# LabJunBMI/E3-invaraint-diffusion-model

Hardware: NVIDIA B200
Metric: denoiser graph-steps/s (forward + reverse-diffusion step per pocket graph; cfg2: 64 pockets x 500 steps, L=128) (higher is better)
Workload: dtype bf16

## Files before the change

e3-invaraint-diffusion-model_b200/csrc/kernels.h:

```cpp
#pragma once
#include "common.cuh"
#include "philox.cuh"

namespace seqdiff {

struct LnResid {
  const float2* stats;
  const float* g;
  const float* b;
};
struct LnOut {
  const float* g;
  const float* b;
  float eps;
  void* h;
  float2* stats;
};
int gemm_16(int M, int N, int K, const void* A, int a_fmt, const void* W, int w_fmt, const float* bias, const float* resid, int epi,
            void* C, int out_kind, cudaStream_t s, int force_bn = 0, const LnResid* ln_resid = nullptr, const LnOut* ln_out = nullptr,
            int split_k = 1);
int gemm_16_tn(int M, int N, int K, const void* At, const void* Bt, int fmt, const float* bias, float* C, cudaStream_t s, int split_k = 1);
int gemm_f32(int M, int N, int K, const float* A, const float* W, const float* bias, const float* resid, int epi, float* C,
             cudaStream_t s);

int make_tmap(const void* ptr, int fmt, int rows, int cols, int box_rows, CUtensorMap* out);
int make_tmap_3d(const void* ptr, int fmt, int batch, int rows, int cols, int box_rows, CUtensorMap* out);

int timestep_embed(const float* timestep, const int* step_ptr, const float* W, int B, int H, float* out, void* out16, int fmt16,
                   cudaStream_t s);
struct EmbedJob {
  const float* x;
  const float* Wt;
  const float* b;
  const float* lnw;
  const float* lnb;
  const float* te;
  float* out32;
  void* outT;
  int M, fin, L;
  const int* src_rows;
  const int* row_graph;
  int cta_begin, cta_count;
};
struct EmbedJobs {
  EmbedJob j[4];
  int n;
  int max_fin;
  float* cat_dst;
  const float* cat_a;
  const float* cat_b;
  int cat_na, cat_nb;
};
template <typename T> int embed_ln_multi(EmbedJobs jobs, float eps, int H, cudaStream_t s);
template <typename T>
int layernorm(const float* in, int M, int H, const float* w, const float* b, float eps, float* out32, T* outT, float2* stats, cudaStream_t s);
template <typename T>
int ln_modulate(const float* in, int M, int H, bool affine_first, const float* lnw, const float* lnb, float eps1, const float* x,
                const T* mod, int mod_div, int chunk0, float* out32, T* outT, cudaStream_t s, const int* row_graph = nullptr);
template <typename T>
int predictor_tail(const T* y, int M, int H, const float* lnw, const float* lnb, float eps, const float* W2, const float* b2,
                   int F, float* logits, cudaStream_t s, const int* dst_rows = nullptr);
template <typename T> int f32_to_16(const float* in, size_t n, T* out, cudaStream_t s);
int transpose_f32(const float* in, int rows, int cols, float* out, cudaStream_t s);
int step_advance(int* step_ptr, cudaStream_t s);

struct AttnPack {
  const int* q_off;
  const int* k_off;
  const int* q_len;
  int q_rows, k_rows;
  int Lk_mask;
};
template <typename T>
int attention(int B, int heads, int Lq, int Lk, const T* q, int ldq, const T* k, int ldk, const T* v, int ldv, const T* dist_emb,
              int P, const float* key_mask, T* out, cudaStream_t s, const AttnPack* pack = nullptr);

int collate(int G, const int* offsets, const uint8_t* lig_mask, const uint8_t* poc_mask, const float* ang, const float* aa, int ext, int L,
            float* lig_ang, float* lig_seq, float* lig_attn, float* rec_ang, float* rec_seq, float* rec_attn, int* lengths, cudaStream_t s);

template <typename T>
int attention_tc(int B, int heads, int Lq, int Lk, const T* q, int ldq, const T* k, int ldk, const T* v, int ldv, const T* dist_emb,
                 int P, const float* key_mask, T* out, cudaStream_t s);
extern unsigned long long* g_attn_trace;
template <typename T>
int attention_pipe(int B, int heads, int Lq, int Lk, const T* q, int ldq, const T* k, int ldk, const T* v, int ldv, const T* dist_emb,
                   int P, const float* key_mask, T* out, cudaStream_t s, const AttnPack* pack = nullptr);
bool attention_bwd_pipe_usable(int Lq, int Lk, const void* dist_emb, float p_drop);
template <typename T>
int attention_bwd_pipe(int B, int heads, int Lq, int Lk, const T* q, int ldq, const T* k, int ldk, const T* v, int ldv, const T* dist_emb, int P,
                       const float* key_mask, DropSpec dr, const T* dout, T* dq, int lddq, T* dk, int lddk, T* dv, int lddv, float* dE, cudaStream_t s,
                       const uint32_t* keep_in = nullptr);
template <typename T>
int attention_pipe_dropout(int B, int heads, int Lq, int Lk, const T* q, int ldq, const T* k, int ldk, const T* v, int ldv, const T* dist_emb,
                           int P, const float* key_mask, DropSpec dr, T* out, cudaStream_t s, uint32_t* keep_out = nullptr);


int reverse_step(const float* q_tables, int n_tab, int B, int L, const float* x_t, const float* logits, int diverse,
                 const float* noise_E, uint64_t seed, uint64_t graph_id0, uint32_t step, const int* step_ptr, float* x_s,
                 uint8_t* idx_out, cudaStream_t s, int* advance = nullptr, const uint64_t* rng = nullptr);
int apply_aa_noise(const float* qtb, int B, int L, const float* x0, const float* noise_E, uint64_t seed, uint64_t graph_id0,
                   uint32_t step, float* x_t, uint8_t* idx_out, cudaStream_t s);
int philox_u32(uint64_t seed, uint64_t graph_id0, uint32_t step, int B, int L, uint32_t* out, cudaStream_t s);

int decode_sequences(int B, int L, const float* final_seq, const float* true_seq, const float* mask, uint8_t* pred_idx, uint8_t* true_idx,
                     int* counts, cudaStream_t s);
int loss_terms(int N, const float* logits, const float* x0, const float* x_t, const float* mask, double* terms, cudaStream_t s,
               double* scratch = nullptr);
size_t loss_terms_scratch_bytes();

int gauss_step(const float* coef, int T, int B, int per_graph, const float* x_t, const float* model_out, const float* noise, uint64_t seed,
               uint64_t graph_id0, int step, const int* step_ptr, float* x_out, float* steps_out, cudaStream_t s, int* advance = nullptr, bool wrap = true,
               const uint64_t* rng = nullptr);

template <typename T> int colsum_add(const T* in, int rows, int cols, float* colsum, cudaStream_t s);
template <typename T> int transpose_colsum(const T* in, int rows, int cols, T* out, float* colsum, cudaStream_t s, int pitch = 0);
template <typename T> int transpose_cast(const float* in, int rows, int cols, T* out, cudaStream_t s);
template <typename T> int act_fwd(const T* z, size_t n, int kind, DropSpec dr, T* a, cudaStream_t s);
template <typename T, typename TG> int act_bwd(const TG* da, const T* z, size_t n, int kind, DropSpec dr, T* dz, cudaStream_t s);
int dropout_add(float* d, const float* resid, size_t n, DropSpec dr, cudaStream_t s);
template <typename T> int grad_cast(const float* g, size_t n, DropSpec dr, T* out, cudaStream_t s);
template <typename T>
int dropout_add_layernorm(float* d, const float* resid, DropSpec dr, int M, int H, const float* w, const float* b, float eps, float* out32, T* outT,
                          uint8_t* keep_bits, cudaStream_t s);
int layernorm_bwd(const float* dh, const float* o, int M, int H, const float* gamma, float eps, float* d_o, float* dgamma, float* dbeta,
                  cudaStream_t s);
template <typename T>
int layernorm_bwd_cast(const float* dh, const float* o, int M, int H, const float* gamma, float eps, float* d_o, float* dgamma, float* dbeta,
                       DropSpec dr, const uint8_t* keep_bits, T* gT, float* dbias, cudaStream_t s);
template <typename T>
int ln_modulate_bwd(const float* dout, const float* in, int M, int H, bool affine_first, const float* lnw, const float* lnb, float eps1,
                    const T* mod, int mod_div, int chunk0, float* din, float* sum_out, T* dmodT, float* dmod32, float* dgamma, float* dbeta,
                    cudaStream_t s);
int embed_bwd(const float* dout, const float* x, int M, int fin, int H, const float* Wt, const float* b, const float* gamma, float eps, DropSpec dr,
              float* dW, float* db, float* dgamma, float* dbeta, cudaStream_t s);
template <typename T>
int predictor_tail_bwd(const float* dlogits, const T* y, int M, int H, const float* gamma, const float* beta, float eps, const float* W2, int F,
                       float* dy, float* dW2, float* db2, float* dgamma, float* dbeta, cudaStream_t s);
int loss_bwd(int N, const float* logits, const float* x0, const float* x_t, const double* terms, float* dlogits, cudaStream_t s);
int adamw_step(float* const* d_w, const int64_t* d_off, int n_slots, size_t total, const float* g, float* m, float* v, float grad_scale,
               float max_norm, float lr, float beta1, float beta2, float eps, float wd, int step, double* d_scratch, float* norm_out, cudaStream_t s);
template <typename T>
int attention_train_fwd(int B, int heads, int Lq, int Lk, const T* q, int ldq, const T* k, int ldk, const T* v, int ldv, const T* dist_emb, int P,
                        const float* key_mask, DropSpec dr, T* out, cudaStream_t s);
template <typename T>
int attention_bwd(int B, int heads, int Lq, int Lk, const T* q, int ldq, const T* k, int ldk, const T* v, int ldv, const T* dist_emb, int P,
                  const float* key_mask, DropSpec dr, const T* dout, T* dq, int lddq, T* dk, int lddk, T* dv, int lddv, float* dE, cudaStream_t s);

template <typename T>
int attention_train_fwd_tc(int B, int heads, int Lq, int Lk, const T* q, int ldq, const T* k, int ldk, const T* v, int ldv, const T* dist_emb, int P,
                           const float* key_mask, DropSpec dr, T* out, cudaStream_t s);
template <typename T>
int attention_bwd_tc(int B, int heads, int Lq, int Lk, const T* q, int ldq, const T* k, int ldk, const T* v, int ldv, const T* dist_emb, int P,
                     const float* key_mask, DropSpec dr, const T* dout, T* dq, int lddq, T* dk, int lddk, T* dv, int lddv, float* dE, cudaStream_t s);

}
```

e3-invaraint-diffusion-model_b200/csrc/model.cu:

```cuda
#include "model.cuh"

#include <mutex>
#include <vector>

#include <cstdio>
#include <cstdlib>
#include <cstring>
#include <type_traits>

namespace seqdiff {

static thread_local std::string g_err;
void set_error(const std::string& msg) { g_err = msg; }
const char* last_error() { return g_err.c_str(); }
std::atomic<uint64_t> g_launches{0};

bool g_profiling = false;
struct ProfMark { const char* tag; cudaEvent_t ev; cudaStream_t s; };
static std::vector<ProfMark> g_marks;
void profile_mark(const char* tag, cudaStream_t s) {
  cudaStreamCaptureStatus st = cudaStreamCaptureStatusNone;
  if (cudaStreamIsCapturing(s, &st) != cudaSuccess || st != cudaStreamCaptureStatusNone) return;
  cudaEvent_t ev;
  if (cudaEventCreate(&ev) != cudaSuccess) return;
  cudaEventRecord(ev, s);
  g_marks.push_back({tag, ev, s});
}
int profile_begin(cudaStream_t s) {
  for (auto& m : g_marks) cudaEventDestroy(m.ev);
  g_marks.clear();
  g_profiling = true;
  profile_mark("__begin__", s);
  return SEQDIFF_OK;
}
int profile_end(char* tags, int tag_stride, float* ms, int* counts, int cap) {
  g_profiling = false;
  if (cudaDeviceSynchronize() != cudaSuccess) return -1;
  std::map<std::string, std::pair<double, int>> agg;
  std::map<cudaStream_t, cudaEvent_t> prev;
  for (auto& m : g_marks) {
    auto it = prev.find(m.s);
    if (it != prev.end() && std::string(m.tag) != "__begin__") {
      float t = 0.f;
      if (cudaEventElapsedTime(&t, it->second, m.ev) == cudaSuccess) {
        auto& a = agg[m.tag];
        a.first += t;
        a.second += 1;
      }
    }
    prev[m.s] = m.ev;
  }
  int n = 0;
  for (auto& kv : agg) {
    if (n >= cap) break;
    std::snprintf(tags + static_cast<size_t>(n) * tag_stride, tag_stride, "%s", kv.first.c_str());
    ms[n] = static_cast<float>(kv.second.first);
    counts[n] = kv.second.second;
    ++n;
  }
  for (auto& m : g_marks) cudaEventDestroy(m.ev);
  g_marks.clear();
  return n;
}

static thread_local int g_pdl_scope = 0;
struct PdlScope {
  const int prev;
  explicit PdlScope(int mode = 1) : prev(g_pdl_scope) { if (mode) g_pdl_scope = mode; }
  ~PdlScope() { g_pdl_scope = prev; }
};
int pdl_scope_exchange(int mode) {
  const int prev = g_pdl_scope;
  g_pdl_scope = mode;
  return prev;
}
static int pdl_auto_mode(long long rows) { return rows <= 2048 ? 1 : (rows <= 32768 ? 3 : 0); }
int pdl_mode() {
  static const int env = [] { const char* e = getenv("SEQDIFF_PDL"); return e ? (e[0] >= '0' && e[0] <= '3' ? e[0] - '0' : 0) : -1; }();
  return env >= 0 ? env : g_pdl_scope;
}
bool pdl_enabled() { return pdl_mode() == 1; }

#ifdef SEQDIFF_DEBUG_BOUNDS
namespace {
struct GuardRec { const void* owner; void* p; };
std::vector<GuardRec> g_guards;
std::mutex g_guard_mu;
constexpr uint32_t kGuardWord = 0xA5C3F00Du;
__global__ void guard_fill_kernel(uint32_t* p) { p[threadIdx.x] = kGuardWord; }
__global__ void guard_check_kernel(uint32_t* const* bands, int n, int* broken) {
  const int i = blockIdx.x;
  if (i < n && bands[i][threadIdx.x] != kGuardWord) atomicAdd(broken, 1);
}
}
int debug_guard_begin(const void* owner) {
  std::lock_guard<std::mutex> g(g_guard_mu);
  size_t w = 0;
  for (size_t i = 0; i < g_guards.size(); ++i)
    if (g_guards[i].owner != owner) g_guards[w++] = g_guards[i];
  g_guards.resize(w);
  return SEQDIFF_OK;
}
int debug_guard_add(const void* owner, void* p, cudaStream_t s) {
  {
    std::lock_guard<std::mutex> g(g_guard_mu);
    g_guards.push_back({owner, p});
  }
  guard_fill_kernel<<<1, 64, 0, s>>>(static_cast<uint32_t*>(p));
  SD_CUDA(cudaGetLastError());
  return SEQDIFF_OK;
}
int debug_guard_check(cudaStream_t s, int* n_bands, int* n_broken) {
  std::vector<uint32_t*> h;
  {
    std::lock_guard<std::mutex> g(g_guard_mu);
    for (auto& r : g_guards) h.push_back(static_cast<uint32_t*>(r.p));
  }
  *n_bands = static_cast<int>(h.size());
  *n_broken = 0;
  if (h.empty()) return SEQDIFF_OK;
  SD_CUDA(cudaDeviceSynchronize());
  if (const char* e = getenv("SEQDIFF_DEBUG_BREAK_GUARD"); e && e[0] == '1') SD_CUDA(cudaMemset(h[h.size() / 2], 0, 4));
  uint32_t** d = nullptr;
  int* cnt = nullptr;
  SD_CUDA(cudaMalloc(reinterpret_cast<void**>(&d), h.size() * sizeof(uint32_t*)));
  SD_CUDA(cudaMalloc(reinterpret_cast<void**>(&cnt), sizeof(int)));
  SD_CUDA(cudaMemcpy(d, h.data(), h.size() * sizeof(uint32_t*), cudaMemcpyHostToDevice));
  SD_CUDA(cudaMemset(cnt, 0, sizeof(int)));
  guard_check_kernel<<<static_cast<unsigned>(h.size()), 64, 0, s>>>(d, static_cast<int>(h.size()), cnt);
  SD_CUDA(cudaGetLastError());
  SD_CUDA(cudaStreamSynchronize(s));
  SD_CUDA(cudaMemcpy(n_broken, cnt, sizeof(int), cudaMemcpyDeviceToHost));
  cudaFree(d);
  cudaFree(cnt);
  return SEQDIFF_OK;
}
#else
int debug_guard_begin(const void*) { return SEQDIFF_OK; }
int debug_guard_add(const void*, void*, cudaStream_t) { return SEQDIFF_OK; }
int debug_guard_check(cudaStream_t, int* n_bands, int* n_broken) { *n_bands = 0; *n_broken = 0; return SEQDIFF_OK; }
#endif

int num_sms() {
  static int n = 0;
  if (n == 0) {
    int dev = 0;
    if (cudaGetDevice(&dev) != cudaSuccess || cudaDeviceGetAttribute(&n, cudaDevAttrMultiProcessorCount, dev) != cudaSuccess || n <= 0)
      n = 148;
  }
  return n;
}

template <typename T> struct Fmt;
template <> struct Fmt<f16> { static constexpr int v = 0; };
template <> struct Fmt<bf16> { static constexpr int v = 1; };
template <> struct Fmt<float> { static constexpr int v = -1; };

template <typename T> static const T* pick(const Wt& w);
template <> const float* pick<float>(const Wt& w) { return w.f; }
template <> const bf16* pick<bf16>(const Wt& w) { return w.h; }
template <> const f16* pick<f16>(const Wt& w) { return w.g; }

static int gemm_T(int, int M, int N, int K, const float* A, const Wt& W, const float* bias, int epi, float* C, cudaStream_t s) {
  return gemm_f32(M, N, K, A, W.f, bias, nullptr, epi, C, s);
}
template <typename T>
static int gemm_T(int wfmt, int M, int N, int K, const T* A, const Wt& W, const float* bias, int epi, T* C, cudaStream_t s) {
  const void* w = wfmt == 1 ? static_cast<const void*>(W.h) : static_cast<const void*>(W.g);
  return gemm_16(M, N, K, A, Fmt<T>::v, w, wfmt, bias, nullptr, epi, C, Fmt<T>::v, s);
}
static int gemm_S(int, int M, int N, int K, const float* A, const Wt& W, const float* bias, const float* resid, float* C, cudaStream_t s) {
  return gemm_f32(M, N, K, A, W.f, bias, resid, 0, C, s);
}
template <typename T>
static int gemm_S(int wfmt, int M, int N, int K, const T* A, const Wt& W, const float* bias, const float* resid, float* C, cudaStream_t s,
                  const LnResid* ln = nullptr, const LnOut* lo = nullptr) {
  const void* w = wfmt == 1 ? static_cast<const void*>(W.h) : static_cast<const void*>(W.g);
  return gemm_16(M, N, K, A, Fmt<T>::v, w, wfmt, bias, resid, 0, C, 2, s, 0, ln, lo);
}
static bool ln_fuse_enabled(int H) {
  static const bool on = [] { const char* e = getenv("SEQDIFF_LN_FUSE"); return e && e[0] == '1'; }();
  return on && (H == 512 || H == 768 || H == 1024);
}
template <typename T>
static int gemm_ln(int wfmt, int M, int H, int K, const T* A, const Wt& W, const float* bias, const float* resid, float* o, const LnResid* lr,
                   const float* ln_w, const float* ln_b, float eps, T* h, float2* stats, cudaStream_t s) {
  if (ln_fuse_enabled(H)) {
    const LnOut lo{ln_w, ln_b, eps, h, stats};
    return gemm_S(wfmt, M, H, K, A, W, bias, resid, o, s, lr, &lo);
  }
  SD_TRY(gemm_S(wfmt, M, H, K, A, W, bias, resid, o, s, lr));
  return layernorm<T>(o, M, H, ln_w, ln_b, eps, nullptr, h, stats, s);
}

__global__ void set_int_kernel(int* p, int v) {
  pdl_trigger();
  pdl_wait();
  *p = v;
}
__global__ void arm_loop_kernel(int* step, int v, uint64_t* rng, uint64_t seed, uint64_t gid0) {
  pdl_trigger();
  pdl_wait();
  step[0] = v;
  step[1] = 0;
  rng[0] = seed;
  rng[1] = gid0;
}

Model::~Model() {
  if (graph_exec) cudaGraphExecDestroy(graph_exec);
  if (loop_stream) cudaStreamDestroy(loop_stream);
  if (ev_in) cudaEventDestroy(ev_in);
  if (ev_out) cudaEventDestroy(ev_out);
  for (void* p : allocs) cudaFree(p);
  for (void* p : packed_allocs) cudaFree(p);
  if (ws) { debug_guard_begin(ws); cudaFree(ws); }
  if (samp_in) { debug_guard_begin(samp_in); cudaFree(samp_in); }
  if (d_tables) cudaFree(d_tables);
  if (d_pack) cudaFree(d_pack);
  if (tws) { debug_guard_begin(tws); cudaFree(tws); }
  if (d_rp_tables) cudaFree(d_rp_tables);
}

void* Model::dalloc(size_t bytes) {
  if (packing && repack_reuse) {
    if (packed_cursor < packed_allocs.size()) return packed_allocs[packed_cursor++];
    return nullptr;
  }
  void* p = nullptr;
  if (cudaMalloc(&p, bytes < 256 ? 256 : bytes) != cudaSuccess) return nullptr;
  (packing ? packed_allocs : allocs).push_back(p);
  return p;
}

static void add_schema(std::map<std::string, RawTensor>& raw, const std::string& name, int64_t numel) {
  RawTensor t;
  t.numel = numel;
  raw[name] = t;
}

int Model::init(const seqdiff_config_t& c, int dev, int arch_) {
  cfg = c;
  device = dev;
  arch = arch_;
  SD_CHECK(c.hidden_size % 256 == 0 && c.hidden_size >= 256 && c.hidden_size <= 1024, "hidden_size must be 256/512/768/1024");
  SD_CHECK(c.num_attention_heads * 64 == c.hidden_size, "head_dim must be 64");
  SD_CHECK(c.intermediate_size % 128 == 0, "intermediate_size must be a multiple of 128");
  SD_CHECK(c.num_hidden_layers >= 1 && c.max_position_embeddings >= 1, "bad layer count / max positions");
  SD_CHECK(c.feature_size >= 1 && c.feature_size <= 32, "feature_size must be in [1,32]");
  SD_CUDA(cudaSetDevice(dev));
  const int64_t H = c.hidden_size, I = c.intermediate_size, P = c.max_position_embeddings;
  add_schema(raw, "timestep_projector.W", H / 2);
  auto emb_schema = [&](const std::string& p, int fin) {
    add_schema(raw, p + ".linear.weight", H * fin);
    add_schema(raw, p + ".linear.bias", H);
    add_schema(raw, p + ".LayerNorm.weight", H);
    add_schema(raw, p + ".LayerNorm.bias", H);
  };
  if (arch == kArchSequence)
    for (const char* side : {"ligand", "receptor"})
      for (auto kv : {std::pair<const char*, int>{"seq", 20}, std::pair<const char*, int>{"angle", 8}})
        emb_schema(std::string(side) + "_" + kv.first + "_embedding", kv.second);
  auto attn = [&](const std::string& p, bool rel) {
    for (const char* n : {"query", "key", "value"}) {
      add_schema(raw, p + ".self." + n + ".weight", H * H);
      add_schema(raw, p + ".self." + n + ".bias", H);
    }
    if (rel && c.relative_key) add_schema(raw, p + ".self.distance_embedding.weight", (2 * P - 1) * 64);
    add_schema(raw, p + ".output.dense.weight", H * H);
    add_schema(raw, p + ".output.dense.bias", H);
    add_schema(raw, p + ".output.LayerNorm.weight", H);
    add_schema(raw, p + ".output.LayerNorm.bias", H);
  };
  auto ffn_schema = [&](const std::string& p) {
    add_schema(raw, p + ".intermediate.dense.weight", I * H);
    add_schema(raw, p + ".intermediate.dense.bias", I);
    add_schema(raw, p + ".output.dense.weight", H * I);
    add_schema(raw, p + ".output.dense.bias", H);
    add_schema(raw, p + ".output.LayerNorm.weight", H);
    add_schema(raw, p + ".output.LayerNorm.bias", H);
  };
  const std::vector<const char*> se_blocks = arch == kArchSequence
                                                 ? std::vector<const char*>{"ligand_feature_emb", "receptor_feature_emb", "decoder_normalize"}
                                                 : std::vector<const char*>{"receptor_emb", "timestep_emb"};
  for (const char* blk : se_blocks) {
    const std::string p = blk;
    add_schema(raw, p + ".adaLN_modulation.0.weight", H * H);
    add_schema(raw, p + ".adaLN_modulation.0.bias", H);
    add_schema(raw, p + ".adaLN_modulation.2.weight", 6 * H * H);
    add_schema(raw, p + ".adaLN_modulation.2.bias", 6 * H);
    attn(p + ".attn", true);
    add_schema(raw, p + ".mlp.0.weight", 4 * H * H);
    add_schema(raw, p + ".mlp.0.bias", 4 * H);
    add_schema(raw, p + ".mlp.3.weight", 4 * H * H);
    add_schema(raw, p + ".mlp.3.bias", H);
  }
  for (int i = 0; i < c.num_hidden_layers; ++i) {
    const std::string p = "decoder.layer." + std::to_string(i);
    attn(p + ".attention", true);
    attn(p + ".crossattention", false);
    ffn_schema(p);
  }
  if (arch == kArchStructure) {
    emb_schema("receptor_seq_emb", 20);
    emb_schema("receptor_angle_emb", c.feature_size);
    emb_schema("ligand_angle_emb", c.feature_size);
    for (int i = 0; i < c.num_hidden_layers; ++i) {
      const std::string p = "encoder.layer." + std::to_string(i);
      attn(p + ".attention", true);
      ffn_schema(p);
    }
  }
  const std::string head = arch == kArchSequence ? "amino_acid_predictor" : "angles_predictor";
  add_schema(raw, head + ".dense1.weight", H * H);
  add_schema(raw, head + ".dense1.bias", H);
  add_schema(raw, head + ".layer_norm.weight", H);
  add_schema(raw, head + ".layer_norm.bias", H);
  add_schema(raw, head + ".dense2.weight", static_cast<int64_t>(c.feature_size) * H);
  add_schema(raw, head + ".dense2.bias", c.feature_size);
  d_step = static_cast<int*>(dalloc(256));
  SD_CHECK(d_step != nullptr, "cudaMalloc failed");
  SD_CUDA(cudaMemset(d_step, 0, 256));
  return SEQDIFF_OK;
}

int Model::set_tensor(const char* name, const float* data, int64_t numel, cudaStream_t s) {
  auto it = raw.find(name);
  if (it == raw.end()) {
    set_error(std::string("unknown tensor name: ") + name);
    return SEQDIFF_ERR_STATE;
  }
  RawTensor& t = it->second;
  if (t.numel != numel) {
    set_error(std::string("size mismatch for ") + name + ": expected " + std::to_string(t.numel) + ", got " + std::to_string(numel));
    return SEQDIFF_ERR_INVALID;
  }
  if (arch == kArchSequence && std::strncmp(name, "receptor_feature_emb.", 21) == 0) {
    t.set = true;
    return SEQDIFF_OK;
  }
  if (!t.ptr) {
    t.ptr = static_cast<float*>(dalloc(static_cast<size_t>(numel) * sizeof(float)));
    SD_CHECK(t.ptr != nullptr, "cudaMalloc failed");
  }
  SD_CUDA(cudaMemcpyAsync(t.ptr, data, static_cast<size_t>(numel) * sizeof(float), cudaMemcpyDefault, s));
  t.set = true;
  finalized = false;
  return SEQDIFF_OK;
}

namespace {
struct RpChunk { const float* src; void* a; void* b; int n, rows, cols, r0; };
__global__ void __launch_bounds__(256) rp_copy_kernel(const RpChunk* __restrict__ tab) {
  const RpChunk c = tab[blockIdx.x];
  float* dst = static_cast<float*>(c.a);
  for (int i = threadIdx.x * 4; i < c.n; i += 1024) {
    if (i + 3 < c.n) *reinterpret_cast<float4*>(dst + i) = *reinterpret_cast<const float4*>(c.src + i);
    else for (int j = i; j < c.n; ++j) dst[j] = c.src[j];
  }
}
__global__ void __launch_bounds__(256) rp_conv_kernel(const RpChunk* __restrict__ tab) {
  const RpChunk c = tab[blockIdx.x];
  bf16* h = static_cast<bf16*>(c.a);
  f16* g = static_cast<f16*>(c.b);
  for (int i = threadIdx.x * 4; i < c.n; i += 1024) {
    if (i + 3 < c.n) {
      const float4 v = *reinterpret_cast<const float4*>(c.src + i);
      *reinterpret_cast<uint2*>(h + i) = make_uint2(pack_bf16x2(v.x, v.y), pack_bf16x2(v.z, v.w));
      *reinterpret_cast<uint2*>(g + i) = make_uint2(pack_f16x2(v.x, v.y), pack_f16x2(v.z, v.w));
    } else {
      for (int j = i; j < c.n; ++j) { h[j] = from_f32<bf16>(c.src[j]); g[j] = from_f32<f16>(c.src[j]); }
    }
  }
}
template <typename T>
__global__ void __launch_bounds__(256) rp_trans_kernel(const RpChunk* __restrict__ tab) {
  __shared__ float tile[64][65];
  const RpChunk c = tab[blockIdx.x];
  T* out = static_cast<T*>(c.a);
  const int r0 = c.r0, c0 = c.n;
  const int tx = threadIdx.x & 63, ty = threadIdx.x >> 6;
#pragma unroll 4
  for (int i = ty; i < 64; i += 4) {
    const int r = r0 + i, cc = c0 + tx;
    tile[i][tx] = (r < c.rows && cc < c.cols) ? c.src[static_cast<size_t>(r) * c.cols + cc] : 0.f;
  }
  __syncthreads();
#pragma unroll 4
  for (int i = ty; i < 64; i += 4) {
    const int cc = c0 + i, r = r0 + tx;
    if (cc < c.cols && r < c.rows) out[static_cast<size_t>(cc) * c.rows + r] = from_f32<T>(tile[tx][i]);
  }
}
}

int Model::repack_fast(cudaStream_t s) {
  constexpr int kChunk = 8192;
  if (!d_rp_tables || rp_table_prec != train_prec) {
    std::vector<RpChunk> tab;
    for (const RpCopy& o : rp_copy)
      for (int64_t off = 0; off < o.n; off += kChunk)
        tab.push_back({o.src + off, o.dst + off, nullptr, static_cast<int>(o.n - off < kChunk ? o.n - off : kChunk), 0, 0, 0});
    rp_n_copy = static_cast<int>(tab.size());
    for (const RpConv& o : rp_conv)
      for (int64_t off = 0; off < o.n; off += kChunk)
        tab.push_back({o.src + off, static_cast<bf16*>(o.h) + off, static_cast<f16*>(o.g) + off, static_cast<int>(o.n - off < kChunk ? o.n - off : kChunk), 0, 0, 0});
    rp_n_conv = static_cast<int>(tab.size()) - rp_n_copy;
    auto tiles = [&](const std::vector<RpTrans>& ops) {
      for (const RpTrans& o : ops)
        for (int r0 = 0; r0 < o.rows; r0 += 64)
          for (int c0 = 0; c0 < o.cols; c0 += 64) tab.push_back({o.src, o.dst, nullptr, c0, o.rows, o.cols, r0});
    };
    const size_t before = tab.size();
    tiles(rp_trans);
    rp_n_trans = static_cast<int>(tab.size() - before);
    tiles(rp_trans_f32);
    rp_n_trans_f32 = static_cast<int>(tab.size() - before) - rp_n_trans;
    if (d_rp_tables) { SD_CUDA(cudaDeviceSynchronize()); SD_CUDA(cudaFree(d_rp_tables)); d_rp_tables = nullptr; }
    SD_CUDA(cudaMalloc(&d_rp_tables, tab.size() * sizeof(RpChunk)));
    SD_CUDA(cudaMemcpyAsync(d_rp_tables, tab.data(), tab.size() * sizeof(RpChunk), cudaMemcpyHostToDevice, s));
    SD_CUDA(cudaStreamSynchronize(s));
    rp_table_prec = train_prec;
  }
  const RpChunk* t = static_cast<const RpChunk*>(d_rp_tables);
  if (rp_n_copy) { SD_CUDA(launch_k(rp_copy_kernel, dim3(rp_n_copy), dim3(256), 0, s, t)); SD_LAUNCHED("repack_copy", s); }
  t += rp_n_copy;
  if (rp_n_conv) { SD_CUDA(launch_k(rp_conv_kernel, dim3(rp_n_conv), dim3(256), 0, s, t)); SD_LAUNCHED("repack_convert", s); }
  t += rp_n_conv;
  if (rp_n_trans) {
    if (train_prec == SEQDIFF_FP32) SD_CUDA(launch_k(rp_trans_kernel<float>, dim3(rp_n_trans), dim3(256), 0, s, t));
    else if (train_prec == SEQDIFF_BF16) SD_CUDA(launch_k(rp_trans_kernel<bf16>, dim3(rp_n_trans), dim3(256), 0, s, t));
    else SD_CUDA(launch_k(rp_trans_kernel<f16>, dim3(rp_n_trans), dim3(256), 0, s, t));
    SD_LAUNCHED("repack_transpose", s);
  }
  t += rp_n_trans;
  if (rp_n_trans_f32) { SD_CUDA(launch_k(rp_trans_kernel<float>, dim3(rp_n_trans_f32), dim3(256), 0, s, t)); SD_LAUNCHED("repack_transpose", s); }
  return SEQDIFF_OK;
}

int Model::finalize(cudaStream_t s) {
  for (auto& kv : raw)
    if (!kv.second.set) {
      set_error("tensor never set: " + kv.first);
      return SEQDIFF_ERR_STATE;
    }
  if (!repack_reuse) {
    if (graph_exec) {
      cudaGraphExecDestroy(graph_exec);
      graph_exec = nullptr;
      graph_key = GraphKey();
    }
    if (!packed_allocs.empty()) {
      SD_CUDA(cudaDeviceSynchronize());
      for (void* p : packed_allocs) cudaFree(p);
      packed_allocs.clear();
    }
  }
  if (repack_reuse && !rp_conv.empty()) return repack_fast(s);
  packed_cursor = 0;
  packing = true;
  rp_copy.clear(); rp_conv.clear(); rp_trans.clear(); rp_trans_f32.clear();
  rp_table_prec = -2;
  const int64_t H = cfg.hidden_size, I = cfg.intermediate_size, P = cfg.max_position_embeddings;
  int rc = SEQDIFF_OK;
  auto R = [&](const std::string& n) -> const float* { return raw.at(n).ptr; };
  auto transposed = [&](Wt& w, int64_t rows, int64_t cols) {
    w.rows = rows;
    w.cols = cols;
    if (train_prec < 0) return;
    const size_t n = static_cast<size_t>(rows) * cols;
    void* t = dalloc(n * (train_prec == SEQDIFF_FP32 ? 4 : 2));
    int r = SEQDIFF_ERR_CUDA;
    if (t) {
      if (train_prec == SEQDIFF_FP32) r = transpose_cast<float>(w.f, static_cast<int>(rows), static_cast<int>(cols), static_cast<float*>(t), s);
      else if (train_prec == SEQDIFF_BF16) r = transpose_cast<bf16>(w.f, static_cast<int>(rows), static_cast<int>(cols), static_cast<bf16*>(t), s);
      else r = transpose_cast<f16>(w.f, static_cast<int>(rows), static_cast<int>(cols), static_cast<f16*>(t), s);
    }
    if (r != SEQDIFF_OK) rc = SEQDIFF_ERR_CUDA;
    w.t = t;
    rp_trans.push_back({w.f, t, static_cast<int>(rows), static_cast<int>(cols)});
  };
  auto both = [&](const float* f, int64_t n) -> Wt {
    Wt w;
    w.f = f;
    bf16* h = static_cast<bf16*>(dalloc(static_cast<size_t>(n) * sizeof(bf16)));
    f16* g = static_cast<f16*>(dalloc(static_cast<size_t>(n) * sizeof(f16)));
    if (!h || !g || f32_to_16<bf16>(f, static_cast<size_t>(n), h, s) != SEQDIFF_OK ||
        f32_to_16<f16>(f, static_cast<size_t>(n), g, s) != SEQDIFF_OK)
      rc = SEQDIFF_ERR_CUDA;
    w.h = h;
    w.g = g;
    rp_conv.push_back({f, h, g, n});
    return w;
  };
  auto stack = [&](const std::vector<const float*>& parts, int64_t each) -> float* {
    float* dst = static_cast<float*>(dalloc(parts.size() * static_cast<size_t>(each) * sizeof(float)));
    if (!dst) { rc = SEQDIFF_ERR_CUDA; return nullptr; }
    for (size_t i = 0; i < parts.size(); ++i) {
      if (cudaMemcpyAsync(dst + i * each, parts[i], static_cast<size_t>(each) * sizeof(float), cudaMemcpyDeviceToDevice, s) != cudaSuccess)
        rc = SEQDIFF_ERR_CUDA;
      rp_copy.push_back({dst + i * each, parts[i], each});
    }
    return dst;
  };
  auto emb = [&](const std::string& p, int fin) -> EmbW {
    EmbW e;
    e.fin = fin;
    float* wt = static_cast<float*>(dalloc(static_cast<size_t>(H) * fin * sizeof(float)));
    if (!wt || transpose_f32(R(p + ".linear.weight"), static_cast<int>(H), fin, wt, s) != SEQDIFF_OK) rc = SEQDIFF_ERR_CUDA;
    e.Wt_ = wt;
    rp_trans_f32.push_back({R(p + ".linear.weight"), wt, static_cast<int>(H), fin});
    e.b = R(p + ".linear.bias");
    e.ln_w = R(p + ".LayerNorm.weight");
    e.ln_b = R(p + ".LayerNorm.bias");
    return e;
  };
  auto attn = [&](const std::string& p, bool self_rel) -> AttnW {
    AttnW a;
    const float* w = stack({R(p + ".self.query.weight"), R(p + ".self.key.weight"), R(p + ".self.value.weight")}, H * H);
    a.qkv = both(w, 3 * H * H);
    transposed(a.qkv, 3 * H, H);
    a.qkv_b = stack({R(p + ".self.query.bias"), R(p + ".self.key.bias"), R(p + ".self.value.bias")}, H);
    if (self_rel && cfg.relative_key) a.E = both(R(p + ".self.distance_embedding.weight"), (2 * P - 1) * 64);
    a.out = both(R(p + ".output.dense.weight"), H * H);
    transposed(a.out, H, H);
    a.out_b = R(p + ".output.dense.bias");
    a.ln_w = R(p + ".output.LayerNorm.weight");
    a.ln_b = R(p + ".output.LayerNorm.bias");
    return a;
  };
  auto se = [&](const std::string& p) -> SEW {
    SEW w;
    w.ada0 = both(R(p + ".adaLN_modulation.0.weight"), H * H);
    transposed(w.ada0, H, H);
    w.ada0_b = R(p + ".adaLN_modulation.0.bias");
    w.ada2 = both(R(p + ".adaLN_modulation.2.weight"), 6 * H * H);
    transposed(w.ada2, 6 * H, H);
    w.ada2_b = R(p + ".adaLN_modulation.2.bias");
    w.attn = attn(p + ".attn", true);
    w.m0 = both(R(p + ".mlp.0.weight"), 4 * H * H);
    transposed(w.m0, 4 * H, H);
    w.m0_b = R(p + ".mlp.0.bias");
    w.m3 = both(R(p + ".mlp.3.weight"), 4 * H * H);
    transposed(w.m3, H, 4 * H);
    w.m3_b = R(p + ".mlp.3.bias");
    return w;
  };
  ts_W = R("timestep_projector.W");
  auto ffn = [&](const std::string& p, LayerW& l) {
    l.inter = both(R(p + ".intermediate.dense.weight"), I * H);
    transposed(l.inter, I, H);
    l.inter_b = R(p + ".intermediate.dense.bias");
    l.outd = both(R(p + ".output.dense.weight"), H * I);
    transposed(l.outd, H, I);
    l.outd_b = R(p + ".output.dense.bias");
    l.oln_w = R(p + ".output.LayerNorm.weight");
    l.oln_b = R(p + ".output.LayerNorm.bias");
  };
  enc_layers.clear();
  if (arch == kArchSequence) {
    lig_seq = emb("ligand_seq_embedding", 20);
    lig_ang = emb("ligand_angle_embedding", 8);
    rec_seq = emb("receptor_seq_embedding", 20);
    rec_ang = emb("receptor_angle_embedding", 8);
    se_lig = se("ligand_feature_emb");
    se_dec = se("decoder_normalize");
  } else {
    rec_seq = emb("receptor_seq_emb", 20);
    rec_ang = emb("receptor_angle_emb", cfg.feature_size);
    lig_ang = emb("ligand_angle_emb", cfg.feature_size);
    se_lig = se("receptor_emb");
    se_dec = se("timestep_emb");
    for (int i = 0; i < cfg.num_hidden_layers; ++i) {
      const std::string p = "encoder.layer." + std::to_string(i);
      LayerW l;
      l.self = attn(p + ".attention", true);
      ffn(p, l);
      enc_layers.push_back(l);
    }
  }
  layers.clear();
  std::vector<const float*> ckv_w, ckv_b;
  for (int i = 0; i < cfg.num_hidden_layers; ++i) {
    const std::string p = "decoder.layer." + std::to_string(i);
    LayerW l;
    l.self = attn(p + ".attention", true);
    l.cq = both(R(p + ".crossattention.self.query.weight"), H * H);
    transposed(l.cq, H, H);
    l.cq_b = R(p + ".crossattention.self.query.bias");
    ckv_w.push_back(R(p + ".crossattention.self.key.weight"));
    ckv_w.push_back(R(p + ".crossattention.self.value.weight"));
    ckv_b.push_back(R(p + ".crossattention.self.key.bias"));
    ckv_b.push_back(R(p + ".crossattention.self.value.bias"));
    l.cout = both(R(p + ".crossattention.output.dense.weight"), H * H);
    transposed(l.cout, H, H);
    l.cout_b = R(p + ".crossattention.output.dense.bias");
    l.cln_w = R(p + ".crossattention.output.LayerNorm.weight");
    l.cln_b = R(p + ".crossattention.output.LayerNorm.bias");
    ffn(p, l);
    layers.push_back(l);
  }
  ckv_all = both(stack(ckv_w, H * H), static_cast<int64_t>(ckv_w.size()) * H * H);
  transposed(ckv_all, static_cast<int64_t>(ckv_w.size()) * H, H);
  ckv_all_b = stack(ckv_b, H);
  const std::string head = arch == kArchSequence ? "amino_acid_predictor" : "angles_predictor";
  p1 = both(R(head + ".dense1.weight"), H * H);
  transposed(p1, H, H);
  p1_b = R(head + ".dense1.bias");
  p_ln_w = R(head + ".layer_norm.weight");
  p_ln_b = R(head + ".layer_norm.bias");
  p2_w = R(head + ".dense2.weight");
  p2_b = R(head + ".dense2.bias");
  packing = false;
  if (rc != SEQDIFF_OK) {
    set_error("finalize: allocation or packing kernel failed");
    return rc;
  }
  finalized = true;
  return SEQDIFF_OK;
}

static size_t align256(size_t b) { return (b + 255) & ~static_cast<size_t>(255); }

size_t Model::workspace_need(int precision, int B, int Ll, int Lr) const {
  const size_t es = precision == SEQDIFF_FP32 ? 4 : 2;
  const size_t dual = precision == SEQDIFF_FP32 ? 4 : 4 + 2;
  const size_t H = cfg.hidden_size, I = cfg.intermediate_size, NL = cfg.num_hidden_layers;
  const size_t Ml = static_cast<size_t>(B) * Ll, Mr = static_cast<size_t>(B) * Lr, Mt = Ml + Mr;
  size_t n = 0;
  n += 2 * align256(static_cast<size_t>(B) * H * 4);
  n += align256((Ml + Mr) * 4);
  n += 3 * (align256(Mt * H * 4) + align256(Mt * H * 2));
  n += 2 * align256(Mt * H * 4);
  n += 3 * align256(Mt * H * es);
  n += align256(Mt * 6 * H * es);
  n += align256(Mt * 3 * H * es);
  n += align256(Mt * 4 * H * es);
  n += align256(Mr * NL * 2 * H * es);
  n += 2 * (align256(Ml * H * 4) + align256(Ml * H * 2));
  n += 2 * align256(Ml * H * es);
  n += align256(Ml * H * 4) + align256(Ml * 3 * 8);
  n += align256(Ml * I * es);
  (void)dual;
  return n + 8192 + 64 * kGuardBytes;
}

int Model::ensure_workspace(size_t bytes) {
  if (bytes <= ws_bytes) return SEQDIFF_OK;
  if (ws) {
    SD_CUDA(cudaDeviceSynchronize());
    debug_guard_begin(ws);
    SD_CUDA(cudaFree(ws));
    ws = nullptr;
    ws_bytes = 0;
  }
  SD_CUDA(cudaMalloc(reinterpret_cast<void**>(&ws), bytes));
  ws_bytes = bytes;
  return SEQDIFF_OK;
}

struct Bump {
  uint8_t* p;
  cudaStream_t gs;
  const void* owner;
  explicit Bump(uint8_t* base, cudaStream_t s = nullptr) : p(base), gs(s), owner(base) { debug_guard_begin(owner); }
  template <typename T> T* take(size_t n) {
    T* r = reinterpret_cast<T*>(p);
    p += align256(n * sizeof(T));
    if (kGuardBytes) {
      debug_guard_add(owner, p, gs);
      p += kGuardBytes;
    }
    return r;
  }
};

template <typename T> struct Act {
  float* s = nullptr;
  T* t = nullptr;
  T* t_out() const { return t; }
};
template <> struct Act<float> {
  float* s = nullptr;
  float* t = nullptr;
  float* t_out() const { return nullptr; }
};
template <typename T> static Act<T> take_act(Bump& bp, size_t n) {
  Act<T> a;
  a.s = bp.take<float>(n);
  a.t = bp.take<T>(n);
  return a;
}
template <> Act<float> take_act<float>(Bump& bp, size_t n) {
  Act<float> a;
  a.s = bp.take<float>(n);
  a.t = a.s;
  return a;
}
template <typename T> static Act<T> offset(const Act<T>& a, size_t n) {
  Act<T> r;
  r.s = a.s + n;
  r.t = a.t + n;
  return r;
}

template <typename T> struct SEBufs {
  T *u, *mod, *qkv, *ctx, *m1;
  float *o, *m2;
  Act<T> x1;
};

template <typename T>
static int se_layer(const Model& m, int wfmt, const SEW& w, const Act<T>& x, const T* c, int Mc, int mod_div, int M,
                    const std::vector<Segment>& segs, const SEBufs<T>& b, const Act<T>& out, cudaStream_t s,
                    const std::vector<AttnPack>* packs = nullptr, const int* row_graph = nullptr) {
  const int H = m.cfg.hidden_size, P = m.cfg.max_position_embeddings, heads = m.cfg.num_attention_heads;
  SD_TRY(gemm_T(wfmt, Mc, H, H, c, w.ada0, w.ada0_b, 2, b.u, s));
  SD_TRY(gemm_T(wfmt, Mc, 6 * H, H, b.u, w.ada2, w.ada2_b, 0, b.mod, s));
  SD_TRY(gemm_T(wfmt, M, 3 * H, H, x.t, w.attn.qkv, w.attn.qkv_b, 0, b.qkv, s));
  for (size_t gi = 0; gi < segs.size(); ++gi) {
    const Segment& g = segs[gi];
    const T* base = b.qkv + static_cast<size_t>(g.row0) * 3 * H;
    SD_TRY(attention<T>(g.B, heads, g.L, g.L, base, 3 * H, base + H, 3 * H, base + 2 * H, 3 * H, pick<T>(w.attn.E), P, g.mask,
                        b.ctx + static_cast<size_t>(g.row0) * H, s, packs ? &(*packs)[gi] : nullptr));
  }
  SD_TRY(gemm_S(wfmt, M, H, H, b.ctx, w.attn.out, w.attn.out_b, x.s, b.o, s));
  SD_TRY(ln_modulate<T>(b.o, M, H, true, w.attn.ln_w, w.attn.ln_b, m.cfg.layer_norm_eps, x.s, b.mod, mod_div, 0, b.x1.s, b.x1.t_out(), s, row_graph));
  SD_TRY(gemm_T(wfmt, M, 4 * H, H, b.x1.t, w.m0, w.m0_b, 1, b.m1, s));
  SD_TRY(gemm_S(wfmt, M, H, 4 * H, b.m1, w.m3, w.m3_b, nullptr, b.m2, s));
  SD_TRY(ln_modulate<T>(b.m2, M, H, false, nullptr, nullptr, 0.f, b.x1.s, b.mod, mod_div, 3, out.s, out.t_out(), s, row_graph));
  return SEQDIFF_OK;
}


template <typename T>
int Model::forward_t(int wfmt, int B, int Ll, int Lr, const float* timestep, const int* step_ptr, const float* x_t,
                     const float* lig_angle, const float* lig_mask, const float* rec_seq_in, const float* rec_angle,
                     const float* rec_mask, float* logits, cudaStream_t s, const PackInfo* pk) {
  constexpr bool k16 = !std::is_same<T, float>::value;
  const int H = cfg.hidden_size, I = cfg.intermediate_size, NL = cfg.num_hidden_layers, heads = cfg.num_attention_heads;
  const int P = cfg.max_position_embeddings;
  const float eps = cfg.layer_norm_eps;
  const int Ml = pk ? pk->Ml : B * Ll, Mr = pk ? pk->Mr : B * Lr, Mt = Ml + Mr;
  const int Mlp = B * Ll, Mrp = B * Lr;
  const size_t MtH = static_cast<size_t>(Mt) * H, MlH = static_cast<size_t>(Ml) * H;
  Bump bp(ws, s);
  float* te = bp.take<float>(static_cast<size_t>(B) * H);
  T* teT = k16 ? bp.take<T>(static_cast<size_t>(B) * H) : reinterpret_cast<T*>(te);
  float* maskcat = bp.take<float>(static_cast<size_t>(Mlp) + Mrp);
  Act<T> x = take_act<T>(bp, MtH);
  Act<T> x2 = take_act<T>(bp, MtH);
  SEBufs<T> sb;
  sb.x1 = take_act<T>(bp, MtH);
  sb.o = bp.take<float>(MtH);
  sb.m2 = bp.take<float>(MtH);
  T* ccat = bp.take<T>(MtH);
  sb.u = bp.take<T>(MtH);
  sb.ctx = bp.take<T>(MtH);
  sb.mod = bp.take<T>(MtH * 6);
  sb.qkv = bp.take<T>(MtH * 3);
  sb.m1 = bp.take<T>(MtH * 4);
  T* kv_all = bp.take<T>(static_cast<size_t>(Mr) * NL * 2 * H);
  Act<T> hbuf[2] = {take_act<T>(bp, MlH), take_act<T>(bp, MlH)};
  float* obuf3 = bp.take<float>(MlH);
  float2* lnstats = bp.take<float2>(3 * static_cast<size_t>(Ml));
  T* cq = bp.take<T>(MlH);
  T* y = bp.take<T>(MlH);
  T* ffn = bp.take<T>(static_cast<size_t>(Ml) * I);

  SD_TRY(timestep_embed(timestep, step_ptr, ts_W, B, H, te, k16 ? static_cast<void*>(teT) : nullptr, Fmt<T>::v, s));
  const Act<T> xr = offset(x, MlH);
  {
    auto job = [&](const float* in, int M, const EmbW& e, const float* te_, int L, float* o32, T* oT, bool lig) {
      EmbedJob jb{};
      jb.x = in; jb.Wt = e.Wt_; jb.b = e.b; jb.lnw = e.ln_w; jb.lnb = e.ln_b; jb.te = te_;
      jb.out32 = o32; jb.outT = oT; jb.M = M; jb.fin = e.fin; jb.L = L;
      if (pk) {
        jb.src_rows = lig ? pk->src_l : pk->src_r;
        jb.row_graph = lig ? pk->graph : pk->graph + pk->Ml;
      }
      return jb;
    };
    EmbedJobs jobs{};
    jobs.n = 4;
    jobs.j[0] = job(x_t, Ml, lig_seq, nullptr, Ll, x.s, x.t_out(), true);
    jobs.j[1] = job(rec_seq_in, Mr, rec_seq, nullptr, Lr, xr.s, xr.t_out(), false);
    jobs.j[2] = job(lig_angle, Ml, lig_ang, te, Ll, k16 ? nullptr : reinterpret_cast<float*>(ccat), k16 ? ccat : nullptr, true);
    jobs.j[3] = job(rec_angle, Mr, rec_ang, te, Lr, k16 ? nullptr : reinterpret_cast<float*>(ccat + MlH), k16 ? ccat + MlH : nullptr, false);
    if (Ll == Lr) {
      jobs.cat_dst = maskcat; jobs.cat_a = lig_mask; jobs.cat_b = rec_mask; jobs.cat_na = Mlp; jobs.cat_nb = Mrp;
    }
    SD_TRY(embed_ln_multi<T>(jobs, eps, H, s));
  }

  std::vector<Segment> segs;
  std::vector<AttnPack> packs;
  AttnPack pk_self{}, pk_cross{};
  if (pk) {
    if (Ll == Lr) {
      segs.push_back({0, 2 * B, pk->max_l > pk->max_r ? pk->max_l : pk->max_r, maskcat});
      packs.push_back(AttnPack{pk->off_cat, pk->off_cat, pk->len_cat, Mt, Mt, Ll});
    } else {
      segs.push_back({0, B, pk->max_l, lig_mask});
      packs.push_back(AttnPack{pk->off_cat, pk->off_cat, pk->len_cat, Mt, Mt, Ll});
      segs.push_back({0, B, pk->max_r, rec_mask});
      packs.push_back(AttnPack{pk->off_cat + B, pk->off_cat + B, pk->len_cat + B, Mt, Mt, Lr});
    }
    pk_self = AttnPack{pk->off_l, pk->off_l, pk->len_l, Ml, Ml, Ll};
    pk_cross = AttnPack{pk->off_l, pk->off_r, pk->len_l, Ml, Mr, Lr};
  } else if (Ll == Lr) {
    segs.push_back({0, 2 * B, Ll, maskcat});
  } else {
    segs.push_back({0, B, Ll, lig_mask});
    segs.push_back({Ml, B, Lr, rec_mask});
  }
  const int Lq_self = pk ? pk->max_l : Ll, Lk_cross = pk ? pk->max_r : Lr;
  const AttnPack* aps = pk ? &pk_self : nullptr;
  const AttnPack* apc = pk ? &pk_cross : nullptr;
  SD_TRY(se_layer<T>(*this, wfmt, se_lig, x, ccat, Mt, 1, Mt, segs, sb, x2, s, pk ? &packs : nullptr, nullptr));
  const T* rec = x2.t + MlH;

  SD_TRY(gemm_T(wfmt, Mr, NL * 2 * H, H, rec, ckv_all, ckv_all_b, 0, kv_all, s));
  Act<T> h = x2;
  if constexpr (k16) {
    float* obuf[3] = {sb.o, sb.m2, obuf3};
    LnResid prev{};
    const float* o_prev = nullptr;
    for (int i = 0; i < NL; ++i) {
      const LayerW& w = layers[i];
      const bool last = i + 1 == NL;
      const Act<T> h1 = hbuf[0], h2 = hbuf[1], h3 = hbuf[0];
      float* oA = obuf[0];
      float* oB = obuf[1];
      float* oC = obuf[2];
      SD_TRY(gemm_T(wfmt, Ml, 3 * H, H, h.t, w.self.qkv, w.self.qkv_b, 0, sb.qkv, s));
      SD_TRY(attention<T>(B, heads, Lq_self, Lq_self, sb.qkv, 3 * H, sb.qkv + H, 3 * H, sb.qkv + 2 * H, 3 * H, pick<T>(w.self.E), P, lig_mask, sb.ctx, s, aps));
      SD_TRY(gemm_ln<T>(wfmt, Ml, H, H, sb.ctx, w.self.out, w.self.out_b, i == 0 ? h.s : o_prev, oA, i == 0 ? nullptr : &prev, w.self.ln_w,
                        w.self.ln_b, eps, h1.t, lnstats, s));
      SD_TRY(gemm_T(wfmt, Ml, H, H, h1.t, w.cq, w.cq_b, 0, cq, s));
      const T* kbase = kv_all + static_cast<size_t>(i) * 2 * H;
      SD_TRY(attention<T>(B, heads, Lq_self, Lk_cross, cq, H, kbase, NL * 2 * H, kbase + H, NL * 2 * H, static_cast<const T*>(nullptr), P, rec_mask, sb.ctx, s, apc));
      const LnResid r1{lnstats, w.self.ln_w, w.self.ln_b};
      SD_TRY(gemm_ln<T>(wfmt, Ml, H, H, sb.ctx, w.cout, w.cout_b, oA, oB, &r1, w.cln_w, w.cln_b, eps, h2.t, lnstats + Ml, s));
      SD_TRY(gemm_T(wfmt, Ml, I, H, h2.t, w.inter, w.inter_b, 1, ffn, s));
      const LnResid r2{lnstats + Ml, w.cln_w, w.cln_b};
      if (last) {
        SD_TRY(gemm_S(wfmt, Ml, H, I, ffn, w.outd, w.outd_b, oB, oC, s, &r2));
        SD_TRY(layernorm<T>(oC, Ml, H, w.oln_w, w.oln_b, eps, h3.s, h3.t, lnstats + 2 * static_cast<size_t>(Ml), s));
      } else {
        SD_TRY(gemm_ln<T>(wfmt, Ml, H, I, ffn, w.outd, w.outd_b, oB, oC, &r2, w.oln_w, w.oln_b, eps, h3.t, lnstats + 2 * static_cast<size_t>(Ml), s));
      }
      prev = LnResid{lnstats + 2 * static_cast<size_t>(Ml), w.oln_w, w.oln_b};
      o_prev = oC;
      h = h3;
    }
  } else {
    for (int i = 0; i < NL; ++i) {
      const LayerW& w = layers[i];
      const Act<T> h1 = hbuf[0], h2 = hbuf[1], h3 = hbuf[0];
      SD_TRY(gemm_T(wfmt, Ml, 3 * H, H, h.t, w.self.qkv, w.self.qkv_b, 0, sb.qkv, s));
      SD_TRY(attention<T>(B, heads, Lq_self, Lq_self, sb.qkv, 3 * H, sb.qkv + H, 3 * H, sb.qkv + 2 * H, 3 * H, pick<T>(w.self.E), P, lig_mask, sb.ctx, s, aps));
      SD_TRY(gemm_S(wfmt, Ml, H, H, sb.ctx, w.self.out, w.self.out_b, h.s, sb.o, s));
      SD_TRY(layernorm<T>(sb.o, Ml, H, w.self.ln_w, w.self.ln_b, eps, h1.s, h1.t_out(), nullptr, s));
      SD_TRY(gemm_T(wfmt, Ml, H, H, h1.t, w.cq, w.cq_b, 0, cq, s));
      const T* kbase = kv_all + static_cast<size_t>(i) * 2 * H;
      SD_TRY(attention<T>(B, heads, Lq_self, Lk_cross, cq, H, kbase, NL * 2 * H, kbase + H, NL * 2 * H, static_cast<const T*>(nullptr), P, rec_mask, sb.ctx, s, apc));
      SD_TRY(gemm_S(wfmt, Ml, H, H, sb.ctx, w.cout, w.cout_b, h1.s, sb.o, s));
      SD_TRY(layernorm<T>(sb.o, Ml, H, w.cln_w, w.cln_b, eps, h2.s, h2.t_out(), nullptr, s));
      SD_TRY(gemm_T(wfmt, Ml, I, H, h2.t, w.inter, w.inter_b, 1, ffn, s));
      SD_TRY(gemm_S(wfmt, Ml, H, I, ffn, w.outd, w.outd_b, h2.s, sb.o, s));
      SD_TRY(layernorm<T>(sb.o, Ml, H, w.oln_w, w.oln_b, eps, h3.s, h3.t_out(), nullptr, s));
      h = h3;
    }
  }

  std::vector<Segment> lseg{{0, B, Lq_self, lig_mask}};
  std::vector<AttnPack> lpack;
  if (pk) lpack.push_back(pk_self);
  SD_TRY(se_layer<T>(*this, wfmt, se_dec, h, teT, B, Ll, Ml, lseg, sb, x, s, pk ? &lpack : nullptr, pk ? pk->graph : nullptr));

  if constexpr (std::is_same<T, bf16>::value) {
    f16* xh = reinterpret_cast<f16*>(sb.ctx);
    f16* yh = reinterpret_cast<f16*>(y);
    SD_TRY(f32_to_16<f16>(x.s, static_cast<size_t>(Ml) * H, xh, s));
    SD_TRY(gemm_16(Ml, H, H, xh, 0, p1.g, 0, p1_b, nullptr, 1, yh, 0, s));
    SD_TRY(predictor_tail<f16>(yh, Ml, H, p_ln_w, p_ln_b, 1e-12f, p2_w, p2_b, cfg.feature_size, logits, s, pk ? pk->src_l : nullptr));
    return SEQDIFF_OK;
  }
  SD_TRY(gemm_T(wfmt, Ml, H, H, x.t, p1, p1_b, 1, y, s));
  SD_TRY(predictor_tail<T>(y, Ml, H, p_ln_w, p_ln_b, 1e-12f, p2_w, p2_b, cfg.feature_size, logits, s, pk ? pk->src_l : nullptr));
  return SEQDIFF_OK;
}

int Model::forward(int precision, int B, int Ll, int Lr, const float* timestep, const int* step_ptr, const float* x_t,
                   const float* lig_angle, const float* lig_mask, const float* rec_seq_in, const float* rec_angle,
                   const float* rec_mask, float* logits, cudaStream_t s, const PackInfo* pk) {
  SD_CHECK(finalized, "model not finalised (seqdiff_model_finalize)");
  SD_CHECK(arch == kArchSequence, "handle holds a structure model: use seqdiff_struct_forward");
  SD_CHECK(!pk || precision != SEQDIFF_FP32, "ragged packing runs in the 16-bit modes");
  SD_CHECK(precision >= SEQDIFF_FP32 && precision <= SEQDIFF_FP16, "unknown precision mode");
  SD_CHECK(B > 0 && Ll > 0 && Lr > 0, "empty batch");
  if (cfg.relative_key) SD_CHECK(Ll <= cfg.max_position_embeddings && Lr <= cfg.max_position_embeddings, "Length exceed");
  SD_CUDA(cudaSetDevice(device));
  SD_TRY(ensure_workspace(workspace_need(precision, B, Ll, Lr)));
  if (g_profiling) profile_mark("__begin__", s);
  const PdlScope pdl_scope(pdl_auto_mode(pk ? static_cast<long long>(pk->Ml) + pk->Mr : static_cast<long long>(B) * (Ll + Lr)));
  switch (precision) {
    case SEQDIFF_FP32:
      return forward_t<float>(1, B, Ll, Lr, timestep, step_ptr, x_t, lig_angle, lig_mask, rec_seq_in, rec_angle, rec_mask, logits, s, nullptr);
    case SEQDIFF_BF16:
      return forward_t<bf16>(1, B, Ll, Lr, timestep, step_ptr, x_t, lig_angle, lig_mask, rec_seq_in, rec_angle, rec_mask, logits, s, pk);
    default:
      return forward_t<f16>(0, B, Ll, Lr, timestep, step_ptr, x_t, lig_angle, lig_mask, rec_seq_in, rec_angle, rec_mask, logits, s, pk);
  }
}

int Model::build_pack(int B, int Ll, int Lr, const float* lig_mask, const float* rec_mask, cudaStream_t s, bool* usable) {
  *usable = false;
  std::vector<float> hl(static_cast<size_t>(B) * Ll), hr(static_cast<size_t>(B) * Lr);
  SD_CUDA(cudaMemcpyAsync(hl.data(), lig_mask, hl.size() * 4, cudaMemcpyDefault, s));
  SD_CUDA(cudaMemcpyAsync(hr.data(), rec_mask, hr.size() * 4, cudaMemcpyDefault, s));
  SD_CUDA(cudaStreamSynchronize(s));
  std::vector<int> len_l(B), len_r(B);
  auto lengths = [&](const std::vector<float>& m, int L, std::vector<int>& len) -> bool {
    for (int b = 0; b < B; ++b) {
      int n = 0;
      while (n < L && m[static_cast<size_t>(b) * L + n] == 1.0f) ++n;
      for (int i = n; i < L; ++i)
        if (m[static_cast<size_t>(b) * L + i] != 0.0f) return false;
      if (n == 0) return false;
      len[b] = n;
    }
    return true;
  };
  if (!lengths(hl, Ll, len_l) || !lengths(hr, Lr, len_r)) return SEQDIFF_OK;
  int Ml = 0, Mr = 0, max_l = 0, max_r = 0;
  std::vector<int> off_l(B), off_r(B);
  for (int b = 0; b < B; ++b) {
    off_l[b] = Ml; Ml += len_l[b];
    off_r[b] = Mr; Mr += len_r[b];
    max_l = len_l[b] > max_l ? len_l[b] : max_l;
    max_r = len_r[b] > max_r ? len_r[b] : max_r;
  }
  std::vector<int> blk;
  blk.reserve(2 * (static_cast<size_t>(Ml) + Mr) + 8 * B);
  for (int b = 0; b < B; ++b) for (int l = 0; l < len_l[b]; ++l) blk.push_back(b * Ll + l);
  for (int b = 0; b < B; ++b) for (int l = 0; l < len_r[b]; ++l) blk.push_back(b * Lr + l);
  for (int b = 0; b < B; ++b) for (int l = 0; l < len_l[b]; ++l) blk.push_back(b);
  for (int b = 0; b < B; ++b) for (int l = 0; l < len_r[b]; ++l) blk.push_back(b);
  for (int b = 0; b < B; ++b) blk.push_back(off_l[b]);
  for (int b = 0; b < B; ++b) blk.push_back(off_r[b]);
  for (int b = 0; b < B; ++b) blk.push_back(len_l[b]);
  for (int b = 0; b < B; ++b) blk.push_back(len_r[b]);
  for (int b = 0; b < B; ++b) blk.push_back(off_l[b]);
  for (int b = 0; b < B; ++b) blk.push_back(Ml + off_r[b]);
  for (int b = 0; b < B; ++b) blk.push_back(len_l[b]);
  for (int b = 0; b < B; ++b) blk.push_back(len_r[b]);
  uint64_t hsh = 1469598103934665603ull;
  for (int v : blk) { hsh ^= static_cast<uint32_t>(v); hsh *= 1099511628211ull; }
  bool fresh = false;
  if (blk.size() > pack_cap) {
    if (d_pack) { SD_CUDA(cudaDeviceSynchronize()); SD_CUDA(cudaFree(d_pack)); d_pack = nullptr; pack_cap = 0; }
    SD_CUDA(cudaMalloc(reinterpret_cast<void**>(&d_pack), blk.size() * sizeof(int)));
    pack_cap = blk.size();
    fresh = true;
  }
  if (fresh || hsh != pack.hash || pack.B != B) {
    SD_CUDA(cudaMemcpyAsync(d_pack, blk.data(), blk.size() * sizeof(int), cudaMemcpyHostToDevice, s));
    SD_CUDA(cudaStreamSynchronize(s));
  }
  PackInfo pi;
  pi.B = B; pi.Ml = Ml; pi.Mr = Mr; pi.max_l = max_l; pi.max_r = max_r; pi.hash = hsh;
  const int* p = d_pack;
  pi.src_l = p; p += Ml;
  pi.src_r = p; p += Mr;
  pi.graph = p; p += Ml + Mr;
  pi.off_l = p; p += B;
  pi.off_r = p; p += B;
  pi.len_l = p; p += B;
  pi.len_r = p; p += B;
  pi.off_cat = p; p += 2 * B;
  pi.len_cat = p;
  pack = pi;
  *usable = true;
  return SEQDIFF_OK;
}

int Model::sample(int precision, int B, int Ll, int Lr, int T, const float* q_tables, const float* x_T, const float* lig_angle,
                  const float* lig_mask, const float* rec_seq_in, const float* rec_angle, const float* rec_mask, int diverse,
                  const float* noise_E, uint64_t seed, uint64_t gid0, float* final_out, cudaStream_t caller, int flags) {
  SD_CHECK(finalized, "model not finalised (seqdiff_model_finalize)");
  SD_CHECK(T >= 1 && B > 0 && Ll > 0 && Lr > 0, "bad sampling arguments");
  SD_CHECK(cfg.feature_size == SEQDIFF_NUM_CLASSES, "sampling needs feature_size == 20");
  SD_CUDA(cudaSetDevice(device));
  if (!loop_stream) {
    SD_CUDA(cudaStreamCreateWithFlags(&loop_stream, cudaStreamNonBlocking));
    SD_CUDA(cudaEventCreateWithFlags(&ev_in, cudaEventDisableTiming));
    SD_CUDA(cudaEventCreateWithFlags(&ev_out, cudaEventDisableTiming));
  }
  cudaStream_t s = loop_stream;
  SD_CUDA(cudaEventRecord(ev_in, caller));
  SD_CUDA(cudaStreamWaitEvent(s, ev_in, 0));
  const size_t Nl = static_cast<size_t>(B) * Ll, Nr = static_cast<size_t>(B) * Lr;
  const size_t need_in = align256(Nl * 20 * 4) * 2 + align256(Nl * 8 * 4) + align256(Nl * 4) + align256(Nr * 20 * 4) +
                         align256(Nr * 8 * 4) + align256(Nr * 4);
  if (need_in + 16 * kGuardBytes > samp_in_bytes) {
    if (samp_in) { SD_CUDA(cudaDeviceSynchronize()); debug_guard_begin(samp_in); SD_CUDA(cudaFree(samp_in)); samp_in = nullptr; samp_in_bytes = 0; }
    SD_CUDA(cudaMalloc(reinterpret_cast<void**>(&samp_in), need_in + 16 * kGuardBytes));
    samp_in_bytes = need_in + 16 * kGuardBytes;
  }
  const size_t tab_floats = static_cast<size_t>(T) * 3 * 400;
  if (tab_floats > tables_cap) {
    if (d_tables) { SD_CUDA(cudaDeviceSynchronize()); SD_CUDA(cudaFree(d_tables)); d_tables = nullptr; tables_cap = 0; }
    SD_CUDA(cudaMalloc(reinterpret_cast<void**>(&d_tables), tab_floats * 4));
    tables_cap = tab_floats;
  }
  SD_TRY(ensure_workspace(workspace_need(precision, B, Ll, Lr)));
  Bump bp(samp_in, s);
  float* x_cur = bp.take<float>(Nl * 20);
  float* logits = bp.take<float>(Nl * 20);
  float* c_lang = bp.take<float>(Nl * 8);
  float* c_lmask = bp.take<float>(Nl);
  float* c_rseq = bp.take<float>(Nr * 20);
  float* c_rang = bp.take<float>(Nr * 8);
  float* c_rmask = bp.take<float>(Nr);
  SD_CUDA(cudaMemcpyAsync(d_tables, q_tables, tab_floats * 4, cudaMemcpyDefault, s));
  SD_CUDA(cudaMemcpyAsync(x_cur, x_T, Nl * 20 * 4, cudaMemcpyDefault, s));
  SD_CUDA(cudaMemcpyAsync(c_lang, lig_angle, Nl * 8 * 4, cudaMemcpyDefault, s));
  SD_CUDA(cudaMemcpyAsync(c_lmask, lig_mask, Nl * 4, cudaMemcpyDefault, s));
  SD_CUDA(cudaMemcpyAsync(c_rseq, rec_seq_in, Nr * 20 * 4, cudaMemcpyDefault, s));
  SD_CUDA(cudaMemcpyAsync(c_rang, rec_angle, Nr * 8 * 4, cudaMemcpyDefault, s));
  SD_CUDA(cudaMemcpyAsync(c_rmask, rec_mask, Nr * 4, cudaMemcpyDefault, s));
  const PackInfo* pk = nullptr;
  if ((flags & 1) && precision != SEQDIFF_FP32) {
    bool usable = false;
    SD_TRY(build_pack(B, Ll, Lr, c_lmask, c_rmask, s, &usable));
    if (usable) {
      pk = &pack;
      SD_CUDA(cudaMemsetAsync(logits, 0, Nl * 20 * 4, s));
    }
  }

  GraphKey key;
  key.pack_hash = pk ? pk->hash : 0;
  key.precision = precision; key.B = B; key.Ll = Ll; key.Lr = Lr; key.diverse = diverse; key.noise = noise_E;
  key.ws_ptr = ws; key.in_ptr = samp_in; key.tab_ptr = d_tables;
  uint64_t* d_rng = reinterpret_cast<uint64_t*>(d_step + 16);
  auto one_step = [&](cudaStream_t st) -> int {
    const PdlScope pdl_scope(pdl_auto_mode(pk ? static_cast<long long>(pk->Ml) + pk->Mr : static_cast<long long>(B) * (Ll + Lr)));
    SD_TRY(forward(precision, B, Ll, Lr, nullptr, d_step, x_cur, c_lang, c_lmask, c_rseq, c_rang, c_rmask, logits, st, pk));
    SD_TRY(reverse_step(d_tables, 1, B, Ll, x_cur, logits, diverse, noise_E, 0, 0, 0, d_step, x_cur, nullptr, st, d_step + 1, d_rng));
    return SEQDIFF_OK;
  };
  if (!graph_exec || !(key == graph_key)) {
    if (graph_exec) { cudaGraphExecDestroy(graph_exec); graph_exec = nullptr; }
    SD_CUDA(launch_k(set_int_kernel, dim3(1), dim3(1), 0, s, d_step, T - 1));
    SD_LAUNCHED("set_int", s);
    SD_TRY(forward(precision, B, Ll, Lr, nullptr, d_step, x_cur, c_lang, c_lmask, c_rseq, c_rang, c_rmask, logits, s, pk));
    SD_CUDA(cudaStreamSynchronize(s));
    cudaGraph_t graph = nullptr;
    const uint64_t l0 = g_launches.load();
    SD_CUDA(cudaStreamBeginCapture(s, cudaStreamCaptureModeThreadLocal));
    const int rc = one_step(s);
    graph_kernels = static_cast<int>(g_launches.load() - l0);
    cudaError_t ce = cudaStreamEndCapture(s, &graph);
    if (rc != SEQDIFF_OK) { if (graph) cudaGraphDestroy(graph); return rc; }
    SD_CUDA(ce);
    ce = cudaGraphInstantiate(&graph_exec, graph, 0);
    cudaGraphDestroy(graph);
    SD_CUDA(ce);
    graph_key = key;
  }
  SD_CUDA(launch_k(arm_loop_kernel, dim3(1), dim3(1), 0, s, d_step, T - 1, d_rng, seed, gid0));
  SD_LAUNCHED("arm_loop", s);
  for (int it = 0; it < T; ++it) SD_CUDA(cudaGraphLaunch(graph_exec, s));
  g_launches.fetch_add(static_cast<uint64_t>(T) * graph_kernels, std::memory_order_relaxed);
  SD_CUDA(cudaMemcpyAsync(final_out, logits, Nl * 20 * 4, cudaMemcpyDefault, s));
  SD_CUDA(cudaEventRecord(ev_out, s));
  SD_CUDA(cudaStreamWaitEvent(caller, ev_out, 0));
  return SEQDIFF_OK;
}

template <typename T>
static int bert_layer_plain(const Model& m, int wfmt, const LayerW& w, bool cross, int B, int Lq, int Lk, const Act<T>& h, const float* q_mask,
                            const float* k_mask, const T* kbase, int ldkv, T* qkv, T* ctx, T* cq, T* ffn, float* o, const Act<T>& h1,
                            const Act<T>& h2, Act<T>* out, cudaStream_t s) {
  const int H = m.cfg.hidden_size, I = m.cfg.intermediate_size, heads = m.cfg.num_attention_heads, P = m.cfg.max_position_embeddings;
  const float eps = m.cfg.layer_norm_eps;
  const int M = B * Lq;
  SD_TRY(gemm_T(wfmt, M, 3 * H, H, h.t, w.self.qkv, w.self.qkv_b, 0, qkv, s));
  SD_TRY(attention<T>(B, heads, Lq, Lq, qkv, 3 * H, qkv + H, 3 * H, qkv + 2 * H, 3 * H, pick<T>(w.self.E), P, q_mask, ctx, s));
  SD_TRY(gemm_S(wfmt, M, H, H, ctx, w.self.out, w.self.out_b, h.s, o, s));
  SD_TRY(layernorm<T>(o, M, H, w.self.ln_w, w.self.ln_b, eps, h1.s, h1.t_out(), nullptr, s));
  Act<T> cur = h1, nxt = h2;
  if (cross) {
    SD_TRY(gemm_T(wfmt, M, H, H, h1.t, w.cq, w.cq_b, 0, cq, s));
    SD_TRY(attention<T>(B, heads, Lq, Lk, cq, H, kbase, ldkv, kbase + H, ldkv, static_cast<const T*>(nullptr), P, k_mask, ctx, s));
    SD_TRY(gemm_S(wfmt, M, H, H, ctx, w.cout, w.cout_b, h1.s, o, s));
    SD_TRY(layernorm<T>(o, M, H, w.cln_w, w.cln_b, eps, h2.s, h2.t_out(), nullptr, s));
    cur = h2;
    nxt = h1;
  }
  SD_TRY(gemm_T(wfmt, M, I, H, cur.t, w.inter, w.inter_b, 1, ffn, s));
  SD_TRY(gemm_S(wfmt, M, H, I, ffn, w.outd, w.outd_b, cur.s, o, s));
  SD_TRY(layernorm<T>(o, M, H, w.oln_w, w.oln_b, eps, nxt.s, nxt.t_out(), nullptr, s));
  *out = nxt;
  return SEQDIFF_OK;
}

template <typename T>
static int bert_stack_lnresid(const Model& m, int wfmt, const std::vector<LayerW>& Ls, bool cross, int B, int Lq, int Lk, const Act<T>& h0,
                              const float* q_mask, const float* k_mask, const T* kv_all, int ldkv, T* qkv, T* ctx, T* cq, T* ffn,
                              float* const (&obuf)[3], float2* lnstats, T* hT0, T* hT1, const T** out, cudaStream_t s) {
  const int H = m.cfg.hidden_size, I = m.cfg.intermediate_size, heads = m.cfg.num_attention_heads, P = m.cfg.max_position_embeddings;
  const float eps = m.cfg.layer_norm_eps;
  const int M = B * Lq;
  float2* stA = lnstats;
  float2* stB = lnstats + M;
  float2* stC = lnstats + 2 * static_cast<size_t>(M);
  LnResid prev{};
  const float* o_prev = nullptr;
  const T* h = h0.t;
  for (size_t i = 0; i < Ls.size(); ++i) {
    const LayerW& w = Ls[i];
    SD_TRY(gemm_T(wfmt, M, 3 * H, H, h, w.self.qkv, w.self.qkv_b, 0, qkv, s));
    SD_TRY(attention<T>(B, heads, Lq, Lq, qkv, 3 * H, qkv + H, 3 * H, qkv + 2 * H, 3 * H, pick<T>(w.self.E), P, q_mask, ctx, s));
    SD_TRY(gemm_ln<T>(wfmt, M, H, H, ctx, w.self.out, w.self.out_b, i == 0 ? h0.s : o_prev, obuf[0], i == 0 ? nullptr : &prev, w.self.ln_w,
                      w.self.ln_b, eps, hT0, stA, s));
    const T* cur = hT0;
    const float* o_cur = obuf[0];
    LnResid rc{stA, w.self.ln_w, w.self.ln_b};
    if (cross) {
      SD_TRY(gemm_T(wfmt, M, H, H, hT0, w.cq, w.cq_b, 0, cq, s));
      const T* kbase = kv_all + i * 2 * static_cast<size_t>(H);
      SD_TRY(attention<T>(B, heads, Lq, Lk, cq, H, kbase, ldkv, kbase + H, ldkv, static_cast<const T*>(nullptr), P, k_mask, ctx, s));
      SD_TRY(gemm_ln<T>(wfmt, M, H, H, ctx, w.cout, w.cout_b, obuf[0], obuf[1], &rc, w.cln_w, w.cln_b, eps, hT1, stB, s));
      cur = hT1;
      o_cur = obuf[1];
      rc = LnResid{stB, w.cln_w, w.cln_b};
    }
    SD_TRY(gemm_T(wfmt, M, I, H, cur, w.inter, w.inter_b, 1, ffn, s));
    T* nxt = cross ? hT0 : hT1;
    SD_TRY(gemm_ln<T>(wfmt, M, H, I, ffn, w.outd, w.outd_b, o_cur, obuf[2], &rc, w.oln_w, w.oln_b, eps, nxt, stC, s));
    prev = LnResid{stC, w.oln_w, w.oln_b};
    o_prev = obuf[2];
    h = nxt;
  }
  *out = h;
  return SEQDIFF_OK;
}

size_t Model::struct_workspace_need(int precision, int B, int Ll, int Lr) const {
  const size_t es = precision == SEQDIFF_FP32 ? 4 : 2;
  const size_t H = cfg.hidden_size, I = cfg.intermediate_size, NL = cfg.num_hidden_layers;
  const size_t Mr = static_cast<size_t>(B) * Lr, Mx = static_cast<size_t>(B) * (Ll > Lr ? Ll : Lr);
  size_t n = align256(Mr * NL * 2 * H * es);
  n += 2 * align256(static_cast<size_t>(B) * H * 4);
  n += 5 * (align256(Mx * H * 4) + align256(Mx * H * 2));
  n += 2 * align256(Mx * H * 4);
  n += 5 * align256(Mx * H * es);
  n += align256(Mx * 6 * H * es) + align256(Mx * 3 * H * es) + align256(Mx * 4 * H * es);
  n += align256(Mx * I * es);
  return n + 8192 + 64 * kGuardBytes;
}

template <typename T>
int Model::struct_forward_t(int wfmt, int B, int Ll, int Lr, const float* timestep, const int* step_ptr, const float* noised,
                            const float* lig_mask, const float* rec_seq_in, const float* rec_angle, const float* rec_mask, float* out,
                            int phases, cudaStream_t s) {
  constexpr bool k16 = !std::is_same<T, float>::value;
  const int H = cfg.hidden_size, I = cfg.intermediate_size, NL = cfg.num_hidden_layers;
  const float eps = cfg.layer_norm_eps;
  const int Ml = B * Ll, Mr = B * Lr, Mx = Ml > Mr ? Ml : Mr;
  const size_t MxH = static_cast<size_t>(Mx) * H;
  Bump bp(ws, s);
  T* kv_all = bp.take<T>(static_cast<size_t>(Mr) * NL * 2 * H);
  float* te = bp.take<float>(static_cast<size_t>(B) * H);
  T* teT = k16 ? bp.take<T>(static_cast<size_t>(B) * H) : reinterpret_cast<T*>(te);
  Act<T> x = take_act<T>(bp, MxH);
  Act<T> x2 = take_act<T>(bp, MxH);
  SEBufs<T> sb;
  sb.x1 = take_act<T>(bp, MxH);
  Act<T> hb[2] = {take_act<T>(bp, MxH), take_act<T>(bp, MxH)};
  sb.o = bp.take<float>(MxH);
  sb.m2 = bp.take<float>(MxH);
  T* cT = bp.take<T>(MxH);
  sb.u = bp.take<T>(MxH);
  sb.ctx = bp.take<T>(MxH);
  T* cq = bp.take<T>(MxH);
  T* y = bp.take<T>(MxH);
  sb.mod = bp.take<T>(MxH * 6);
  sb.qkv = bp.take<T>(MxH * 3);
  sb.m1 = bp.take<T>(MxH * 4);
  T* ffn = bp.take<T>(static_cast<size_t>(Mx) * I);
  auto job = [&](const float* in, int M, const EmbW& e, int L, float* o32, T* oT) {
    EmbedJob jb{};
    jb.x = in; jb.Wt = e.Wt_; jb.b = e.b; jb.lnw = e.ln_w; jb.lnb = e.ln_b; jb.te = nullptr;
    jb.out32 = o32; jb.outT = oT; jb.M = M; jb.fin = e.fin; jb.L = L;
    return jb;
  };

  if (phases & 1) {
    EmbedJobs jobs{};
    jobs.n = 2;
    jobs.j[0] = job(rec_angle, Mr, rec_ang, Lr, x.s, x.t_out());
    jobs.j[1] = job(rec_seq_in, Mr, rec_seq, Lr, k16 ? nullptr : reinterpret_cast<float*>(cT), k16 ? cT : nullptr);
    SD_TRY(embed_ln_multi<T>(jobs, eps, H, s));
    std::vector<Segment> rseg{{0, B, Lr, rec_mask}};
    SD_TRY(se_layer<T>(*this, wfmt, se_lig, x, cT, Mr, 1, Mr, rseg, sb, x2, s));
    const T* enc_out = nullptr;
    if constexpr (k16) {
      float* const obuf[3] = {sb.o, sb.m2, hb[0].s};
      SD_TRY(bert_stack_lnresid<T>(*this, wfmt, enc_layers, false, B, Lr, Lr, x2, rec_mask, nullptr, nullptr, 0, sb.qkv, sb.ctx, cq, ffn, obuf,
                                   reinterpret_cast<float2*>(hb[1].s), hb[0].t, hb[1].t, &enc_out, s));
    } else {
      Act<T> h = x2;
      for (int i = 0; i < NL; ++i) {
        Act<T> nh;
        SD_TRY(bert_layer_plain<T>(*this, wfmt, enc_layers[i], false, B, Lr, Lr, h, rec_mask, nullptr, nullptr, 0, sb.qkv, sb.ctx, cq, ffn, sb.o,
                                   hb[0], hb[1], &nh, s));
        h = nh;
      }
      enc_out = h.t;
    }
    SD_TRY(gemm_T(wfmt, Mr, NL * 2 * H, H, enc_out, ckv_all, ckv_all_b, 0, kv_all, s));
  }

  if (!(phases & 2)) return SEQDIFF_OK;
  SD_TRY(timestep_embed(timestep, step_ptr, ts_W, B, H, te, k16 ? static_cast<void*>(teT) : nullptr, Fmt<T>::v, s));
  {
    EmbedJobs jobs{};
    jobs.n = 1;
    jobs.j[0] = job(noised, Ml, lig_ang, Ll, x.s, x.t_out());
    SD_TRY(embed_ln_multi<T>(jobs, eps, H, s));
  }
  std::vector<Segment> lseg{{0, B, Ll, lig_mask}};
  SD_TRY(se_layer<T>(*this, wfmt, se_dec, x, teT, B, Ll, Ml, lseg, sb, x2, s));
  const T* dec_out = nullptr;
  if constexpr (k16) {
    float* const obuf[3] = {sb.o, sb.m2, hb[0].s};
    SD_TRY(bert_stack_lnresid<T>(*this, wfmt, layers, true, B, Ll, Lr, x2, lig_mask, rec_mask, kv_all, NL * 2 * H, sb.qkv, sb.ctx, cq, ffn, obuf,
                                 reinterpret_cast<float2*>(hb[1].s), hb[0].t, hb[1].t, &dec_out, s));
  } else {
    Act<T> h = x2;
    for (int i = 0; i < NL; ++i) {
      Act<T> nh;
      const T* kbase = kv_all + static_cast<size_t>(i) * 2 * H;
      SD_TRY(bert_layer_plain<T>(*this, wfmt, layers[i], true, B, Ll, Lr, h, lig_mask, rec_mask, kbase, NL * 2 * H, sb.qkv, sb.ctx, cq, ffn, sb.o,
                                 hb[0], hb[1], &nh, s));
      h = nh;
    }
    dec_out = h.t;
  }
  SD_TRY(gemm_T(wfmt, Ml, H, H, dec_out, p1, p1_b, 1, y, s));
  SD_TRY(predictor_tail<T>(y, Ml, H, p_ln_w, p_ln_b, 1e-12f, p2_w, p2_b, cfg.feature_size, out, s));
  return SEQDIFF_OK;
}

int Model::struct_forward(int precision, int B, int Ll, int Lr, const float* timestep, const int* step_ptr, const float* noised,
                          const float* lig_mask, const float* rec_seq_in, const float* rec_angle, const float* rec_mask, float* out,
                          int phases, cudaStream_t s) {
  SD_CHECK(finalized, "model not finalised (seqdiff_model_finalize)");
  SD_CHECK(arch == kArchStructure, "handle holds a sequence model: use seqdiff_forward");
  const PdlScope pdl_on(3);
  SD_CHECK(precision >= SEQDIFF_FP32 && precision <= SEQDIFF_FP16, "unknown precision mode");
  SD_CHECK(B > 0 && Ll > 0 && Lr > 0, "empty batch");
  if (cfg.relative_key) SD_CHECK(Ll <= cfg.max_position_embeddings && Lr <= cfg.max_position_embeddings, "Length exceed");
  SD_CUDA(cudaSetDevice(device));
  SD_TRY(ensure_workspace(struct_workspace_need(precision, B, Ll, Lr)));
  if (g_profiling) profile_mark("__begin__", s);
  switch (precision) {
    case SEQDIFF_FP32:
      return struct_forward_t<float>(1, B, Ll, Lr, timestep, step_ptr, noised, lig_mask, rec_seq_in, rec_angle, rec_mask, out, phases, s);
    case SEQDIFF_BF16:
      return struct_forward_t<bf16>(1, B, Ll, Lr, timestep, step_ptr, noised, lig_mask, rec_seq_in, rec_angle, rec_mask, out, phases, s);
    default:
      return struct_forward_t<f16>(0, B, Ll, Lr, timestep, step_ptr, noised, lig_mask, rec_seq_in, rec_angle, rec_mask, out, phases, s);
  }
}

int Model::struct_sample(int precision, int B, int Ll, int Lr, int T, const float* coef_steps, const float* x_T, const float* lig_mask,
                         const float* rec_seq_in, const float* rec_angle, const float* rec_mask, const float* noise_steps, uint64_t seed,
                         uint64_t gid0, float* steps_out, float* final_out, cudaStream_t caller) {
  SD_CHECK(finalized, "model not finalised (seqdiff_model_finalize)");
  SD_CHECK(arch == kArchStructure, "handle holds a sequence model: use seqdiff_sample");
  const PdlScope pdl_on(3);
  SD_CHECK(T >= 1 && B > 0 && Ll > 0 && Lr > 0, "bad sampling arguments");
  SD_CUDA(cudaSetDevice(device));
  if (!loop_stream) {
    SD_CUDA(cudaStreamCreateWithFlags(&loop_stream, cudaStreamNonBlocking));
    SD_CUDA(cudaEventCreateWithFlags(&ev_in, cudaEventDisableTiming));
    SD_CUDA(cudaEventCreateWithFlags(&ev_out, cudaEventDisableTiming));
  }
  cudaStream_t s = loop_stream;
  SD_CUDA(cudaEventRecord(ev_in, caller));
  SD_CUDA(cudaStreamWaitEvent(s, ev_in, 0));
  const int F = cfg.feature_size;
  const size_t Nl = static_cast<size_t>(B) * Ll, Nr = static_cast<size_t>(B) * Lr;
  const size_t need_in = align256(Nl * F * 4) * 2 + align256(Nl * 4) + align256(Nr * 20 * 4) + align256(Nr * F * 4) + align256(Nr * 4);
  if (need_in + 16 * kGuardBytes > samp_in_bytes) {
    if (samp_in) { SD_CUDA(cudaDeviceSynchronize()); debug_guard_begin(samp_in); SD_CUDA(cudaFree(samp_in)); samp_in = nullptr; samp_in_bytes = 0; }
    SD_CUDA(cudaMalloc(reinterpret_cast<void**>(&samp_in), need_in + 16 * kGuardBytes));
    samp_in_bytes = need_in + 16 * kGuardBytes;
  }
  const size_t tab_floats = static_cast<size_t>(T) * 4;
  if (tab_floats > tables_cap) {
    if (d_tables) { SD_CUDA(cudaDeviceSynchronize()); SD_CUDA(cudaFree(d_tables)); d_tables = nullptr; tables_cap = 0; }
    SD_CUDA(cudaMalloc(reinterpret_cast<void**>(&d_tables), tab_floats * 4));
    tables_cap = tab_floats;
  }
  SD_TRY(ensure_workspace(struct_workspace_need(precision, B, Ll, Lr)));
  Bump bp(samp_in, s);
  float* x_cur = bp.take<float>(Nl * F);
  float* mout = bp.take<float>(Nl * F);
  float* c_lmask = bp.take<float>(Nl);
  float* c_rseq = bp.take<float>(Nr * 20);
  float* c_rang = bp.take<float>(Nr * F);
  float* c_rmask = bp.take<float>(Nr);
  SD_CUDA(cudaMemcpyAsync(d_tables, coef_steps, tab_floats * 4, cudaMemcpyDefault, s));
  SD_CUDA(cudaMemcpyAsync(x_cur, x_T, Nl * F * 4, cudaMemcpyDefault, s));
  SD_CUDA(cudaMemcpyAsync(c_lmask, lig_mask, Nl * 4, cudaMemcpyDefault, s));
  SD_CUDA(cudaMemcpyAsync(c_rseq, rec_seq_in, Nr * 20 * 4, cudaMemcpyDefault, s));
  SD_CUDA(cudaMemcpyAsync(c_rang, rec_angle, Nr * F * 4, cudaMemcpyDefault, s));
  SD_CUDA(cudaMemcpyAsync(c_rmask, rec_mask, Nr * 4, cudaMemcpyDefault, s));

  GraphKey key;
  key.precision = precision; key.B = B; key.Ll = Ll; key.Lr = Lr; key.diverse = 0; key.noise = noise_steps;
  key.ws_ptr = ws; key.in_ptr = samp_in; key.tab_ptr = d_tables; key.aux_ptr = steps_out; key.T = T;
  uint64_t* d_rng = reinterpret_cast<uint64_t*>(d_step + 16);
  SD_CUDA(launch_k(arm_loop_kernel, dim3(1), dim3(1), 0, s, d_step, T - 1, d_rng, seed, gid0));
  SD_LAUNCHED("arm_loop", s);
  const bool cached = graph_exec && key == graph_key;
  SD_TRY(struct_forward(precision, B, Ll, Lr, nullptr, d_step, x_cur, c_lmask, c_rseq, c_rang, c_rmask, mout, cached ? 1 : 3, s));
  auto one_step = [&](cudaStream_t st) -> int {
    SD_TRY(struct_forward(precision, B, Ll, Lr, nullptr, d_step, x_cur, c_lmask, c_rseq, c_rang, c_rmask, mout, 2, st));
    SD_TRY(gauss_step(d_tables, T, B, Ll * F, x_cur, mout, noise_steps, 0, 0, 0, d_step, x_cur, steps_out, st, d_step + 1, true, d_rng));
    return SEQDIFF_OK;
  };
  if (!cached) {
    if (graph_exec) { cudaGraphExecDestroy(graph_exec); graph_exec = nullptr; }
    SD_CUDA(cudaStreamSynchronize(s));
    cudaGraph_t graph = nullptr;
    const uint64_t l0 = g_launches.load();
    SD_CUDA(cudaStreamBeginCapture(s, cudaStreamCaptureModeThreadLocal));
    const int rc = one_step(s);
    graph_kernels = static_cast<int>(g_launches.load() - l0);
    cudaError_t ce = cudaStreamEndCapture(s, &graph);
    if (rc != SEQDIFF_OK) { if (graph) cudaGraphDestroy(graph); return rc; }
    SD_CUDA(ce);
    ce = cudaGraphInstantiate(&graph_exec, graph, 0);
    cudaGraphDestroy(graph);
    SD_CUDA(ce);
    graph_key = key;
  }
  for (int it = 0; it < T; ++it) SD_CUDA(cudaGraphLaunch(graph_exec, s));
  g_launches.fetch_add(static_cast<uint64_t>(T) * graph_kernels, std::memory_order_relaxed);
  SD_CUDA(cudaMemcpyAsync(final_out, x_cur, Nl * F * 4, cudaMemcpyDefault, s));
  SD_CUDA(cudaEventRecord(ev_out, s));
  SD_CUDA(cudaStreamWaitEvent(caller, ev_out, 0));
  return SEQDIFF_OK;
}

}
```

e3-invaraint-diffusion-model_b200/csrc/model.cuh:

```cuda
#pragma once
#include <map>
#include <string>
#include <vector>

#include "kernels.h"

namespace seqdiff {

struct Wt {
  const float* f = nullptr;
  const bf16* h = nullptr;
  const f16* g = nullptr;
  const void* t = nullptr;
  int64_t rows = 0, cols = 0;
};

struct AttnW {
  Wt qkv;
  const float* qkv_b = nullptr;
  Wt E;
  Wt out;
  const float *out_b = nullptr, *ln_w = nullptr, *ln_b = nullptr;
};
struct SEW {
  Wt ada0, ada2, m0, m3;
  const float *ada0_b = nullptr, *ada2_b = nullptr, *m0_b = nullptr, *m3_b = nullptr;
  AttnW attn;
};
struct LayerW {
  AttnW self;
  Wt cq, cout, inter, outd;
  const float *cq_b = nullptr, *cout_b = nullptr, *cln_w = nullptr, *cln_b = nullptr;
  const float *inter_b = nullptr, *outd_b = nullptr, *oln_w = nullptr, *oln_b = nullptr;
};
struct EmbW {
  const float *Wt_ = nullptr, *b = nullptr, *ln_w = nullptr, *ln_b = nullptr;
  int fin = 0;
};

struct RawTensor {
  float* ptr = nullptr;
  int64_t numel = 0;
  bool set = false;
};

struct ParamSlot {
  std::string name;
  float* w = nullptr;
  int64_t numel = 0, off = 0;
};

struct TrainArgs {
  int precision, B, Ll, Lr;
  const float *t_norm, *x_t, *x0, *lig_angle, *lig_mask, *rec_seq, *rec_angle, *rec_mask;
  float p_hidden, p_attn;
  uint64_t seed;
  uint32_t step;
  float* grads;
  double* terms;
  float* logits_out;
};

struct Segment {
  int row0, B, L;
  const float* mask;
};

int profile_begin(cudaStream_t s);
int profile_end(char* tags, int tag_stride, float* ms, int* counts, int cap);

struct PackInfo {
  int B = 0, Ml = 0, Mr = 0;
  int max_l = 0, max_r = 0;
  const int* src_l = nullptr;
  const int* src_r = nullptr;
  const int* graph = nullptr;
  const int* off_l = nullptr;
  const int* off_r = nullptr;
  const int* len_l = nullptr;
  const int* len_r = nullptr;
  const int* off_cat = nullptr;
  const int* len_cat = nullptr;
  uint64_t hash = 0;
};

enum Arch { kArchSequence = 0, kArchStructure = 1 };

struct Model {
  seqdiff_config_t cfg{};
  int arch = kArchSequence;
  int device = 0;
  bool finalized = false;
  std::map<std::string, RawTensor> raw;
  std::vector<void*> allocs;
  std::vector<void*> packed_allocs;
  bool packing = false;

  EmbW lig_seq, lig_ang, rec_seq, rec_ang;
  SEW se_lig, se_dec;
  std::vector<LayerW> layers;
  std::vector<LayerW> enc_layers;
  Wt ckv_all;
  const float* ckv_all_b = nullptr;
  Wt p1;
  const float *p1_b = nullptr, *p_ln_w = nullptr, *p_ln_b = nullptr, *p2_w = nullptr, *p2_b = nullptr, *ts_W = nullptr;

  uint8_t* ws = nullptr;
  size_t ws_bytes = 0;

  int* d_step = nullptr;
  float* d_tables = nullptr;
  size_t tables_cap = 0;
  uint8_t* samp_in = nullptr;
  size_t samp_in_bytes = 0;
  cudaGraphExec_t graph_exec = nullptr;
  int graph_kernels = 0;
  cudaStream_t loop_stream = nullptr;
  cudaEvent_t ev_in = nullptr, ev_out = nullptr;
  struct GraphKey {
    int precision = -1, B = 0, Ll = 0, Lr = 0, diverse = 0;
    const float* noise = nullptr;
    const void* ws_ptr = nullptr;
    const void* in_ptr = nullptr;
    const void* tab_ptr = nullptr;
    const void* aux_ptr = nullptr;
    int T = 0;
    uint64_t pack_hash = 0;
    bool operator==(const GraphKey& o) const {
      return pack_hash == o.pack_hash && aux_ptr == o.aux_ptr && T == o.T && precision == o.precision && B == o.B && Ll == o.Ll && Lr == o.Lr && diverse == o.diverse && noise == o.noise &&
             ws_ptr == o.ws_ptr && in_ptr == o.in_ptr && tab_ptr == o.tab_ptr;
    }
  } graph_key;

  ~Model();
  int init(const seqdiff_config_t& c, int dev, int arch_ = kArchSequence);
  int set_tensor(const char* name, const float* data, int64_t numel, cudaStream_t s);
  int finalize(cudaStream_t s);
  int forward(int precision, int B, int Ll, int Lr, const float* timestep, const int* step_ptr, const float* x_t,
              const float* lig_angle, const float* lig_mask, const float* rec_seq, const float* rec_angle, const float* rec_mask,
              float* logits, cudaStream_t s, const PackInfo* pk = nullptr);
  int sample(int precision, int B, int Ll, int Lr, int T, const float* q_tables, const float* x_T, const float* lig_angle,
             const float* lig_mask, const float* rec_seq, const float* rec_angle, const float* rec_mask, int diverse,
             const float* noise_E, uint64_t seed, uint64_t gid0, float* final_out, cudaStream_t s, int flags = 0);
  int* d_pack = nullptr;
  size_t pack_cap = 0;
  PackInfo pack;
  int build_pack(int B, int Ll, int Lr, const float* lig_mask, const float* rec_mask, cudaStream_t s, bool* usable);

  std::vector<ParamSlot> slots;
  std::map<std::string, int> slot_of;
  int64_t train_total = 0;
  std::vector<int64_t> grad_bucket_bounds;
  std::vector<cudaEvent_t> bucket_events;
  int train_prec = -1;
  bool repack_reuse = false;
  size_t packed_cursor = 0;
  struct RpCopy { float* dst; const float* src; int64_t n; };
  struct RpConv { const float* src; void* h; void* g; int64_t n; };
  struct RpTrans { const float* src; void* dst; int rows, cols; };
  std::vector<RpCopy> rp_copy;
  std::vector<RpConv> rp_conv;
  std::vector<RpTrans> rp_trans, rp_trans_f32;
  void* d_rp_tables = nullptr;
  int rp_n_copy = 0, rp_n_conv = 0, rp_n_trans = 0, rp_n_trans_f32 = 0, rp_table_prec = -2;
  int repack_fast(cudaStream_t s);
  float** d_slot_w = nullptr;
  int64_t* d_slot_off = nullptr;
  double* d_opt_scratch = nullptr;
  float* d_zero_bias = nullptr;
  uint8_t* tws = nullptr;
  size_t tws_bytes = 0;
  int build_slots();
  int64_t train_param_count();
  int train_step(const TrainArgs& a, cudaStream_t s);
  int adamw(const float* grads, float* m, float* v, float grad_scale, float max_norm, float lr, float beta1, float beta2, float eps, float wd,
            int step, float* norm_out, cudaStream_t s);
  int get_tensor(const char* name, float* out, int64_t numel, cudaStream_t s);
  template <typename T> int train_t(int wfmt, const TrainArgs& a, cudaStream_t s);

  int struct_forward(int precision, int B, int Ll, int Lr, const float* timestep, const int* step_ptr, const float* noised_angles,
                     const float* lig_mask, const float* rec_seq, const float* rec_angle, const float* rec_mask, float* out, int phases,
                     cudaStream_t s);
  int struct_sample(int precision, int B, int Ll, int Lr, int T, const float* coef_steps, const float* x_T, const float* lig_mask,
                    const float* rec_seq, const float* rec_angle, const float* rec_mask, const float* noise_steps, uint64_t seed,
                    uint64_t gid0, float* steps_out, float* final_out, cudaStream_t s);

 public:
  void* dalloc(size_t bytes);
  size_t struct_workspace_need(int precision, int B, int Ll, int Lr) const;
  template <typename T>
  int struct_forward_t(int wfmt, int B, int Ll, int Lr, const float* timestep, const int* step_ptr, const float* noised_angles,
                       const float* lig_mask, const float* rec_seq, const float* rec_angle, const float* rec_mask, float* out, int phases,
                       cudaStream_t s);
  size_t workspace_need(int precision, int B, int Ll, int Lr) const;
  int ensure_workspace(size_t bytes);
  template <typename T>
  int forward_t(int wfmt, int B, int Ll, int Lr, const float* timestep, const int* step_ptr, const float* x_t, const float* lig_angle,
                const float* lig_mask, const float* rec_seq, const float* rec_angle, const float* rec_mask, float* logits,
                cudaStream_t s, const PackInfo* pk);
};

}
```

e3-invaraint-diffusion-model_b200/csrc/rowwise.cu:

```cuda
#include <cstdlib>

#include "common.cuh"
#include "kernels.h"

namespace seqdiff {

constexpr int kRowThreads = 256;
constexpr int kEmbedTok = 2;

template <typename T, int VPL>
__device__ __forceinline__ void load_row(const T* __restrict__ row, int lane, float (&v)[VPL][8]) {
#pragma unroll
  for (int i = 0; i < VPL; ++i) load8<T>(row + (i * 32 + lane) * 8, v[i]);
}
template <typename T, int VPL>
__device__ __forceinline__ void store_row(T* __restrict__ row, int lane, const float (&v)[VPL][8]) {
#pragma unroll
  for (int i = 0; i < VPL; ++i) store8<T>(row + (i * 32 + lane) * 8, v[i]);
}
template <int VPL>
__device__ __forceinline__ void row_stats(const float (&v)[VPL][8], int H, float eps, float& mean, float& rstd) {
  float s = 0.f;
#pragma unroll
  for (int i = 0; i < VPL; ++i)
#pragma unroll
    for (int j = 0; j < 8; ++j) s += v[i][j];
  mean = warp_sum(s) / static_cast<float>(H);
  float q = 0.f;
#pragma unroll
  for (int i = 0; i < VPL; ++i)
#pragma unroll
    for (int j = 0; j < 8; ++j) {
      const float d = v[i][j] - mean;
      q = fmaf(d, d, q);
    }
  const float var = warp_sum(q) / static_cast<float>(H);
  rstd = 1.0f / sqrtf(var + eps);
}

__global__ void timestep_embed_kernel(const float* __restrict__ timestep, const int* __restrict__ step_ptr,
                                      const float* __restrict__ W, int B, int H, float* __restrict__ out, void* __restrict__ out16, int fmt16) {
  pdl_trigger();
  pdl_wait();
  const int half = H / 2;
  const int i = blockIdx.x * blockDim.x + threadIdx.x;
  if (i >= B * half) return;
  const int b = i / half, j = i % half;
  const float t = step_ptr ? static_cast<float>(*step_ptr) : timestep[b];
  const float x = __fmul_rn(__fmul_rn(__fmul_rn(t, W[j]), 2.0f), 3.14159274101257324f);
  const float sv = sinf(x), cv = cosf(x);
  out[static_cast<size_t>(b) * H + j] = sv;
  out[static_cast<size_t>(b) * H + half + j] = cv;
  if (out16) {
    if (fmt16 == 1) {
      bf16* o = static_cast<bf16*>(out16);
      o[static_cast<size_t>(b) * H + j] = from_f32<bf16>(sv);
      o[static_cast<size_t>(b) * H + half + j] = from_f32<bf16>(cv);
    } else {
      f16* o = static_cast<f16*>(out16);
      o[static_cast<size_t>(b) * H + j] = from_f32<f16>(sv);
      o[static_cast<size_t>(b) * H + half + j] = from_f32<f16>(cv);
    }
  }
}

int timestep_embed(const float* timestep, const int* step_ptr, const float* W, int B, int H, float* out, void* out16, int fmt16,
                   cudaStream_t s) {
  const int n = B * (H / 2);
  SD_CUDA(launch_k(timestep_embed_kernel, dim3(ceil_div(n, 128)), dim3(128), 0, s, timestep, step_ptr, W, B, H, out, out16, fmt16));
  SD_LAUNCHED("timestep_embed", s);
  return SEQDIFF_OK;
}

template <typename T, int VPL>
__global__ void __launch_bounds__(kRowThreads, 2) embed_ln_multi_kernel(const __grid_constant__ EmbedJobs jobs, float eps, int H) {
  extern __shared__ float4 sW4[];
  float* sW = reinterpret_cast<float*>(sW4);
  int q = 0;
#pragma unroll
  for (int t = 1; t < 4; ++t)
    if (t < jobs.n && static_cast<int>(blockIdx.x) >= jobs.j[t].cta_begin) q = t;
  const EmbedJob& job = jobs.j[q];
  const int fin = job.fin, M = job.M;
  for (int i = threadIdx.x; i < fin * H / 4; i += kRowThreads) sW4[i] = __ldg(reinterpret_cast<const float4*>(job.Wt) + i);
  pdl_trigger();
  pdl_wait();
  if (jobs.cat_dst) {
    for (int i = blockIdx.x * kRowThreads + threadIdx.x; i < jobs.cat_na + jobs.cat_nb; i += gridDim.x * kRowThreads)
      jobs.cat_dst[i] = i < jobs.cat_na ? __ldg(jobs.cat_a + i) : __ldg(jobs.cat_b + (i - jobs.cat_na));
  }
  __syncthreads();
  constexpr int TOK = kEmbedTok;
  const int lane = threadIdx.x & 31, warp = threadIdx.x >> 5;
  const int cta_local = static_cast<int>(blockIdx.x) - job.cta_begin;
  T* outT = static_cast<T*>(job.outT);
  float* sx = sW + static_cast<size_t>(jobs.max_fin) * H + warp * (2 * TOK * 32);
  const int gstep = job.cta_count * (kRowThreads / 32);
  auto fetch_x = [&](int grp_n, int buf) {
    if (job.src_rows) {
      for (int i = lane; i < TOK * fin; i += 32) {
        const int r = grp_n * TOK + i / fin;
        sx[buf * TOK * 32 + i] = r < M ? __ldg(job.x + static_cast<size_t>(__ldg(job.src_rows + r)) * fin + (i % fin)) : 0.f;
      }
      return;
    }
    const size_t base = static_cast<size_t>(grp_n) * TOK * fin;
    const size_t lim = static_cast<size_t>(M) * fin;
    for (int i = lane; i < TOK * fin; i += 32) sx[buf * TOK * 32 + i] = (base + i < lim) ? __ldg(job.x + base + i) : 0.f;
  };
  int xb = 0;
  {
    const int g0 = cta_local * (kRowThreads / 32) + warp;
    if (g0 * TOK < M) fetch_x(g0, 0);
    __syncwarp();
  }
  for (int grp = cta_local * (kRowThreads / 32) + warp; grp * TOK < M; grp += gstep, xb ^= 1) {
    const int tok0 = grp * TOK;
    if ((grp + gstep) * TOK < M) fetch_x(grp + gstep, xb ^ 1);
    const float* xs = sx + xb * TOK * 32;
    float acc[TOK][VPL][8];
#pragma unroll
    for (int t = 0; t < TOK; ++t)
#pragma unroll
      for (int i = 0; i < VPL; ++i)
#pragma unroll
        for (int jj = 0; jj < 8; ++jj) acc[t][i][jj] = 0.f;
    for (int k = 0; k < fin; ++k) {
      float xv[TOK];
      bool any = false;
#pragma unroll
      for (int t = 0; t < TOK; ++t) {
        xv[t] = xs[t * fin + k];
        any |= xv[t] != 0.f;
      }
      if (!any) continue;
#pragma unroll
      for (int i = 0; i < VPL; ++i) {
        float w[8];
        load8<float>(sW + static_cast<size_t>(k) * H + (i * 32 + lane) * 8, w);
#pragma unroll
        for (int t = 0; t < TOK; ++t)
#pragma unroll
          for (int jj = 0; jj < 8; ++jj) acc[t][i][jj] = fmaf(xv[t], w[jj], acc[t][i][jj]);
      }
    }
#pragma unroll
    for (int t = 0; t < TOK; ++t) {
      if (tok0 + t >= M) break;
      float v[VPL][8];
#pragma unroll
      for (int i = 0; i < VPL; ++i) {
        float b8[8];
        load8<float>(job.b + (i * 32 + lane) * 8, b8);
#pragma unroll
        for (int jj = 0; jj < 8; ++jj) v[i][jj] = acc[t][i][jj] + b8[jj];
      }
      float mean, rstd;
      row_stats<VPL>(v, H, eps, mean, rstd);
      const float* terow = job.te ? job.te + static_cast<size_t>(job.row_graph ? __ldg(job.row_graph + tok0 + t) : (tok0 + t) / job.L) * H : nullptr;
#pragma unroll
      for (int i = 0; i < VPL; ++i) {
        float g8[8], b8[8];
        load8<float>(job.lnw + (i * 32 + lane) * 8, g8);
        load8<float>(job.lnb + (i * 32 + lane) * 8, b8);
#pragma unroll
        for (int jj = 0; jj < 8; ++jj) v[i][jj] = (v[i][jj] - mean) * rstd * g8[jj] + b8[jj];
        if (terow) {
          float t8[8];
          load8<float>(terow + (i * 32 + lane) * 8, t8);
#pragma unroll
          for (int jj = 0; jj < 8; ++jj) v[i][jj] += t8[jj];
        }
      }
      if (job.out32) store_row<float, VPL>(job.out32 + static_cast<size_t>(tok0 + t) * H, lane, v);
      if (outT) store_row<T, VPL>(outT + static_cast<size_t>(tok0 + t) * H, lane, v);
    }
    __syncwarp();
  }
}

#define SD_VPL_DISPATCH(H_, ...)                                        \
  switch ((H_) / 256) {                                                  \
    case 1: { constexpr int VPL = 1; __VA_ARGS__; } break;                      \
    case 2: { constexpr int VPL = 2; __VA_ARGS__; } break;                      \
    case 3: { constexpr int VPL = 3; __VA_ARGS__; } break;                      \
    case 4: { constexpr int VPL = 4; __VA_ARGS__; } break;                      \
    default: set_error("hidden_size must be 256, 512, 768 or 1024"); return SEQDIFF_ERR_INVALID; \
  }

template <typename T>
int embed_ln_multi(EmbedJobs jobs, float eps, int H, cudaStream_t s) {
  SD_CHECK(H % 256 == 0, "hidden_size must be a multiple of 256");
  SD_CHECK(jobs.n >= 1 && jobs.n <= 4, "1..4 embedding jobs per launch");
  long total = 0;
  int max_fin = 0;
  for (int q = 0; q < jobs.n; ++q) {
    SD_CHECK(jobs.j[q].M > 0 && jobs.j[q].fin > 0 && jobs.j[q].fin <= 32 && jobs.j[q].L > 0, "bad embedding job");
    total += jobs.j[q].M;
    max_fin = jobs.j[q].fin > max_fin ? jobs.j[q].fin : max_fin;
  }
  const int budget = 2 * num_sms();
  int begin = 0;
  for (int q = 0; q < jobs.n; ++q) {
    int c = static_cast<int>(static_cast<long>(budget) * jobs.j[q].M / total);
    const int need = ceil_div(jobs.j[q].M, kEmbedTok * (kRowThreads / 32));
    if (c < 1) c = 1;
    if (c > need) c = need;
    jobs.j[q].cta_begin = begin;
    jobs.j[q].cta_count = c;
    begin += c;
  }
  jobs.max_fin = max_fin;
  const size_t smem = static_cast<size_t>(max_fin) * H * sizeof(float) + (kRowThreads / 32) * 2 * kEmbedTok * 32 * sizeof(float);
#define SD_EMBED_LAUNCH()                                                                                                          \
  {                                                                                                                                \
    auto kfn = embed_ln_multi_kernel<T, VPL>;                                                                                      \
    static bool configured = false;                                                                                                \
    if (!configured) {                                                                                                             \
      SD_CUDA(cudaFuncSetAttribute(kfn, cudaFuncAttributeMaxDynamicSharedMemorySize, 32 * 1024 * 4 + 8192));                       \
      configured = true;                                                                                                           \
    }                                                                                                                              \
    SD_CUDA(launch_k(kfn, dim3(begin), dim3(kRowThreads), smem, s, jobs, eps, H));                                                 \
  }
  SD_VPL_DISPATCH(H, SD_EMBED_LAUNCH());
#undef SD_EMBED_LAUNCH
  SD_LAUNCHED("embed_ln", s);
  return SEQDIFF_OK;
}
template int embed_ln_multi<float>(EmbedJobs, float, int, cudaStream_t);
template int embed_ln_multi<bf16>(EmbedJobs, float, int, cudaStream_t);
template int embed_ln_multi<f16>(EmbedJobs, float, int, cudaStream_t);

template <typename T, int VPL, int THREADS = kRowThreads, int RPW = 1>
__global__ void __launch_bounds__(THREADS) layernorm_kernel(const float* __restrict__ in, int M, int H, const float* __restrict__ w,
                                                            const float* __restrict__ b, float eps, float* __restrict__ out32,
                                                            T* __restrict__ outT, float2* __restrict__ stats) {
  pdl_trigger();
  pdl_wait();
  const int lane = threadIdx.x & 31;
  const int row0 = ((blockIdx.x * THREADS + threadIdx.x) >> 5) * RPW;
  if (row0 >= M) return;
  float v[RPW][VPL][8];
#pragma unroll
  for (int r = 0; r < RPW; ++r)
    if (row0 + r < M) load_row<float, VPL>(in + static_cast<size_t>(row0 + r) * H, lane, v[r]);
#pragma unroll
  for (int r = 0; r < RPW; ++r) {
    const int row = row0 + r;
    if (row >= M) break;
    float mean, rstd;
    row_stats<VPL>(v[r], H, eps, mean, rstd);
    if (stats && lane == 0) stats[row] = make_float2(mean, rstd);
#pragma unroll
    for (int i = 0; i < VPL; ++i) {
      float g8[8], b8[8];
      load8<float>(w + (i * 32 + lane) * 8, g8);
      load8<float>(b + (i * 32 + lane) * 8, b8);
#pragma unroll
      for (int j = 0; j < 8; ++j) v[r][i][j] = (v[r][i][j] - mean) * rstd * g8[j] + b8[j];
    }
    if (out32) store_row<float, VPL>(out32 + static_cast<size_t>(row) * H, lane, v[r]);
    if (outT) store_row<T, VPL>(outT + static_cast<size_t>(row) * H, lane, v[r]);
  }
}

template <typename T>
int layernorm(const float* in, int M, int H, const float* w, const float* b, float eps, float* out32, T* outT, float2* stats, cudaStream_t s) {
  static const int var = [] { const char* e = getenv("SEQDIFF_LN_VAR"); return e ? atoi(e) : 2561; }();
#define SD_LN_LAUNCH(TH_, RPW_)                                                                                                           \
  {                                                                                                                                       \
    const int grid = ceil_div(ceil_div(M, RPW_) * 32, TH_);                                                                               \
    SD_VPL_DISPATCH(H, SD_CUDA(launch_k(layernorm_kernel<T, VPL, TH_, RPW_>, dim3(grid), dim3(TH_), 0, s, in, M, H, w, b, eps, out32, outT, stats))); \
  }
  switch (var) {
    case 1281: SD_LN_LAUNCH(128, 1); break;
    case 5121: SD_LN_LAUNCH(512, 1); break;
    case 2562: SD_LN_LAUNCH(256, 2); break;
    case 1282: SD_LN_LAUNCH(128, 2); break;
    case 641: SD_LN_LAUNCH(64, 1); break;
    default: SD_LN_LAUNCH(256, 1); break;
  }
#undef SD_LN_LAUNCH
  SD_LAUNCHED("layernorm", s);
  return SEQDIFF_OK;
}
#define SD_INST_LN(T) template int layernorm<T>(const float*, int, int, const float*, const float*, float, float*, T*, float2*, cudaStream_t)
SD_INST_LN(float);
SD_INST_LN(bf16);
SD_INST_LN(f16);

template <typename T, int VPL, bool AFFINE_FIRST>
__global__ void __launch_bounds__(kRowThreads) ln_modulate_kernel(const float* __restrict__ in, int M, int H, const float* __restrict__ lnw,
                                                                  const float* __restrict__ lnb, float eps1, const float* __restrict__ x,
                                                                  const T* __restrict__ mod, int mod_div, int chunk0,
                                                                  float* __restrict__ out32, T* __restrict__ outT, const int* __restrict__ row_graph) {
  pdl_trigger();
  pdl_wait();
  const int lane = threadIdx.x & 31;
  const int row = (blockIdx.x * kRowThreads + threadIdx.x) >> 5;
  if (row >= M) return;
  float v[VPL][8];
  load_row<float, VPL>(in + static_cast<size_t>(row) * H, lane, v);
  float mean, rstd;
  if (AFFINE_FIRST) {
    row_stats<VPL>(v, H, eps1, mean, rstd);
#pragma unroll
    for (int i = 0; i < VPL; ++i) {
      float g8[8], b8[8];
      load8<float>(lnw + (i * 32 + lane) * 8, g8);
      load8<float>(lnb + (i * 32 + lane) * 8, b8);
#pragma unroll
      for (int j = 0; j < 8; ++j) v[i][j] = (v[i][j] - mean) * rstd * g8[j] + b8[j];
    }
  }
  row_stats<VPL>(v, H, 1e-5f, mean, rstd);
  SD_DEV_ASSERT(!row_graph || __ldg(row_graph + row) >= 0);
  const T* mrow = mod + static_cast<size_t>(row_graph ? __ldg(row_graph + row) : row / mod_div) * (6 * H);
  const float* xrow = x + static_cast<size_t>(row) * H;
#pragma unroll
  for (int i = 0; i < VPL; ++i) {
    const int e = (i * 32 + lane) * 8;
    float sh[8], sc[8], gt[8], xr[8];
    load8<T>(mrow + (chunk0 + 0) * H + e, sh);
    load8<T>(mrow + (chunk0 + 1) * H + e, sc);
    load8<T>(mrow + (chunk0 + 2) * H + e, gt);
    load8<float>(xrow + e, xr);
#pragma unroll
    for (int j = 0; j < 8; ++j) {
      const float n = (v[i][j] - mean) * rstd;
      v[i][j] = xr[j] + gt[j] * (n * (1.0f + sc[j]) + sh[j]);
    }
  }
  if (out32) store_row<float, VPL>(out32 + static_cast<size_t>(row) * H, lane, v);
  if (outT) store_row<T, VPL>(outT + static_cast<size_t>(row) * H, lane, v);
}

template <typename T>
int ln_modulate(const float* in, int M, int H, bool affine_first, const float* lnw, const float* lnb, float eps1, const float* x,
                const T* mod, int mod_div, int chunk0, float* out32, T* outT, cudaStream_t s, const int* row_graph) {
  const int grid = ceil_div(M * 32, kRowThreads);
  if (affine_first) {
    SD_VPL_DISPATCH(H, SD_CUDA(launch_k(ln_modulate_kernel<T, VPL, true>, dim3(grid), dim3(kRowThreads), 0, s, in, M, H, lnw, lnb, eps1, x, mod, mod_div, chunk0, out32, outT, row_graph)));
  } else {
    SD_VPL_DISPATCH(H, SD_CUDA(launch_k(ln_modulate_kernel<T, VPL, false>, dim3(grid), dim3(kRowThreads), 0, s, in, M, H, lnw, lnb, eps1, x, mod, mod_div, chunk0, out32, outT, row_graph)));
  }
  SD_LAUNCHED("ln_modulate", s);
  return SEQDIFF_OK;
}
#define SD_INST_LNMOD(T) \
  template int ln_modulate<T>(const float*, int, int, bool, const float*, const float*, float, const float*, const T*, int, int, float*, T*, cudaStream_t, const int*)
SD_INST_LNMOD(float);
SD_INST_LNMOD(bf16);
SD_INST_LNMOD(f16);

template <typename T, int VPL>
__global__ void __launch_bounds__(kRowThreads) predictor_tail_kernel(const T* __restrict__ y, int M, int H, const float* __restrict__ lnw,
                                                                     const float* __restrict__ lnb, float eps,
                                                                     const float* __restrict__ W2, const float* __restrict__ b2, int F,
                                                                     float* __restrict__ logits, const int* __restrict__ dst_rows) {
  extern __shared__ float4 sW4[];
  float* sW = reinterpret_cast<float*>(sW4);
  for (int i = threadIdx.x; i < F * H / 4; i += kRowThreads) sW4[i] = __ldg(reinterpret_cast<const float4*>(W2) + i);
  float* sG = sW + static_cast<size_t>(F) * H;
  for (int i = threadIdx.x; i < H; i += kRowThreads) {
    sG[i] = __ldg(lnw + i);
    sG[H + i] = __ldg(lnb + i);
  }
  pdl_trigger();
  pdl_wait();
  __syncthreads();
  constexpr int ROWS = 4;
  const int lane = threadIdx.x & 31, warp = threadIdx.x >> 5;
  const float bias_f = lane < F ? b2[lane] : 0.f;
  for (int grp = blockIdx.x * (kRowThreads / 32) + warp; grp * ROWS < M; grp += gridDim.x * (kRowThreads / 32)) {
    const int row0 = grp * ROWS;
    float v[ROWS][VPL][8];
#pragma unroll
    for (int r = 0; r < ROWS; ++r) {
      const int row = row0 + r < M ? row0 + r : M - 1;
      load_row<T, VPL>(y + static_cast<size_t>(row) * H, lane, v[r]);
      float mean, rstd;
      row_stats<VPL>(v[r], H, eps, mean, rstd);
#pragma unroll
      for (int i = 0; i < VPL; ++i) {
        float g8[8], be8[8];
        load8<float>(sG + (i * 32 + lane) * 8, g8);
        load8<float>(sG + H + (i * 32 + lane) * 8, be8);
#pragma unroll
        for (int jj = 0; jj < 8; ++jj) v[r][i][jj] = (v[r][i][jj] - mean) * rstd * g8[jj] + be8[jj];
      }
    }
    float mine[ROWS];
#pragma unroll
    for (int r = 0; r < ROWS; ++r) mine[r] = 0.f;
    for (int f = 0; f < F; ++f) {
      float p[ROWS];
#pragma unroll
      for (int r = 0; r < ROWS; ++r) p[r] = 0.f;
#pragma unroll
      for (int i = 0; i < VPL; ++i) {
        float w[8];
        load8<float>(sW + static_cast<size_t>(f) * H + (i * 32 + lane) * 8, w);
#pragma unroll
        for (int r = 0; r < ROWS; ++r)
#pragma unroll
          for (int jj = 0; jj < 8; ++jj) p[r] = fmaf(v[r][i][jj], w[jj], p[r]);
      }
#pragma unroll
      for (int r = 0; r < ROWS; ++r) {
        p[r] = warp_sum(p[r]);
        if (lane == f) mine[r] = p[r] + bias_f;
      }
    }
#pragma unroll
    for (int r = 0; r < ROWS; ++r)
      if (lane < F && row0 + r < M) logits[static_cast<size_t>(dst_rows ? __ldg(dst_rows + row0 + r) : row0 + r) * F + lane] = mine[r];
  }
}

template <typename T>
int predictor_tail(const T* y, int M, int H, const float* lnw, const float* lnb, float eps, const float* W2, const float* b2, int F,
                   float* logits, cudaStream_t s, const int* dst_rows) {
  SD_CHECK(F <= 32, "feature_size > 32 not supported");
  const int need = ceil_div(M, 4 * (kRowThreads / 32));
  const int grid = need < num_sms() ? need : num_sms();
  const size_t smem = (static_cast<size_t>(F) + 2) * H * sizeof(float);
#define SD_PRED_LAUNCH()                                                                                              \
  {                                                                                                                   \
    auto kfn = predictor_tail_kernel<T, VPL>;                                                                         \
    static bool configured = false;                                                                                   \
    if (!configured) {                                                                                                \
      SD_CUDA(cudaFuncSetAttribute(kfn, cudaFuncAttributeMaxDynamicSharedMemorySize, 34 * 1024 * 4));                 \
      configured = true;                                                                                              \
    }                                                                                                                 \
    SD_CUDA(launch_k(kfn, dim3(grid), dim3(kRowThreads), smem, s, y, M, H, lnw, lnb, eps, W2, b2, F, logits, dst_rows)); \
  }
  SD_VPL_DISPATCH(H, SD_PRED_LAUNCH());
#undef SD_PRED_LAUNCH
  SD_LAUNCHED("predictor_tail", s);
  return SEQDIFF_OK;
}
template int predictor_tail<float>(const float*, int, int, const float*, const float*, float, const float*, const float*, int, float*, cudaStream_t, const int*);
template int predictor_tail<bf16>(const bf16*, int, int, const float*, const float*, float, const float*, const float*, int, float*, cudaStream_t, const int*);
template int predictor_tail<f16>(const f16*, int, int, const float*, const float*, float, const float*, const float*, int, float*, cudaStream_t, const int*);

template <typename T>
__global__ void f32_to_16_kernel(const float* __restrict__ in, size_t n, T* __restrict__ out) {
  pdl_trigger();
  pdl_wait();
  size_t i = (static_cast<size_t>(blockIdx.x) * blockDim.x + threadIdx.x);
  const size_t stride = static_cast<size_t>(gridDim.x) * blockDim.x;
  const size_t n4 = ((reinterpret_cast<uintptr_t>(in) & 15) == 0 && (reinterpret_cast<uintptr_t>(out) & 7) == 0) ? n / 4 : 0;
  for (size_t v = i; v < n4; v += stride) {
    const float4 a = *reinterpret_cast<const float4*>(in + 4 * v);
    *reinterpret_cast<uint2*>(out + 4 * v) = make_uint2(pack2<T>(a.x, a.y), pack2<T>(a.z, a.w));
  }
  for (i += 4 * n4; i < n; i += stride) out[i] = from_f32<T>(in[i]);
}
template <typename T>
int f32_to_16(const float* in, size_t n, T* out, cudaStream_t s) {
  if (n == 0) return SEQDIFF_OK;
  size_t blocks = (n + 255) / 256;
  if (blocks > 4096) blocks = 4096;
  SD_CUDA(launch_k(f32_to_16_kernel<T>, dim3(static_cast<int>(blocks)), dim3(256), 0, s, in, n, out));
  SD_LAUNCHED("f32_to_16", s);
  return SEQDIFF_OK;
}
template int f32_to_16<bf16>(const float*, size_t, bf16*, cudaStream_t);
template int f32_to_16<f16>(const float*, size_t, f16*, cudaStream_t);

__global__ void transpose_f32_kernel(const float* __restrict__ in, int rows, int cols, float* __restrict__ out) {
  pdl_trigger();
  pdl_wait();
  const int i = blockIdx.x * blockDim.x + threadIdx.x;
  if (i >= rows * cols) return;
  const int r = i / cols, c = i % cols;
  out[static_cast<size_t>(c) * rows + r] = in[i];
}
int transpose_f32(const float* in, int rows, int cols, float* out, cudaStream_t s) {
  SD_CUDA(launch_k(transpose_f32_kernel, dim3(ceil_div(rows * cols, 256)), dim3(256), 0, s, in, rows, cols, out));
  SD_LAUNCHED("transpose_f32", s);
  return SEQDIFF_OK;
}

__global__ void step_advance_kernel(int* p) {
  pdl_trigger();
  pdl_wait();
  *p -= 1;
}
int step_advance(int* step_ptr, cudaStream_t s) {
  SD_CUDA(launch_k(step_advance_kernel, dim3(1), dim3(1), 0, s, step_ptr));
  SD_LAUNCHED("step_advance", s);
  return SEQDIFF_OK;
}

}
```

Baseline: 33660.

## Hoist sampling-loop invariants (receptor embedding/attention, timestep modulation) out of the reverse loop

Precomputes per-sampling-call invariants before the reverse-diffusion loop: the receptor sequence embedding and its self-attention output in the ligand SE layer, timestep embeddings for all T steps, and the decoder adaLN modulation tables indexed by the device step counter. Each forward step then runs QKV/out-proj GEMMs only on ligand rows, and ln_modulate reads the precomputed receptor rows through a split source. This removes repeated receptor-side and timestep MLP work each step, at the cost of extra workspace, a more complex graph key and one-time setup per sample call.

```diff
diff --git a/e3-invaraint-diffusion-model_b200/csrc/kernels.h b/e3-invaraint-diffusion-model_b200/csrc/kernels.h
--- a/e3-invaraint-diffusion-model_b200/csrc/kernels.h
+++ b/e3-invaraint-diffusion-model_b200/csrc/kernels.h
@@ -40,6 +40,7 @@
   int M, fin, L;
   const int* src_rows;
   const int* row_graph;
+  const int* te_row;
   int cta_begin, cta_count;
 };
 struct EmbedJobs {
@@ -56,7 +57,8 @@
 int layernorm(const float* in, int M, int H, const float* w, const float* b, float eps, float* out32, T* outT, float2* stats, cudaStream_t s);
 template <typename T>
 int ln_modulate(const float* in, int M, int H, bool affine_first, const float* lnw, const float* lnb, float eps1, const float* x,
-                const T* mod, int mod_div, int chunk0, float* out32, T* outT, cudaStream_t s, const int* row_graph = nullptr);
+                const T* mod, int mod_div, int chunk0, float* out32, T* outT, cudaStream_t s, const int* row_graph = nullptr,
+                const int* mod_row = nullptr, int split = 0, const float* in_hi = nullptr, const float* x_hi = nullptr);
 template <typename T>
 int predictor_tail(const T* y, int M, int H, const float* lnw, const float* lnb, float eps, const float* W2, const float* b2,
                    int F, float* logits, cudaStream_t s, const int* dst_rows = nullptr);
diff --git a/e3-invaraint-diffusion-model_b200/csrc/model.cu b/e3-invaraint-diffusion-model_b200/csrc/model.cu
--- a/e3-invaraint-diffusion-model_b200/csrc/model.cu
+++ b/e3-invaraint-diffusion-model_b200/csrc/model.cu
@@ -216,6 +216,7 @@
   for (void* p : packed_allocs) cudaFree(p);
   if (ws) { debug_guard_begin(ws); cudaFree(ws); }
   if (samp_in) { debug_guard_begin(samp_in); cudaFree(samp_in); }
+  if (samp_inv) { debug_guard_begin(samp_inv); cudaFree(samp_inv); }
   if (d_tables) cudaFree(d_tables);
   if (d_pack) cudaFree(d_pack);
   if (tws) { debug_guard_begin(tws); cudaFree(tws); }
@@ -710,70 +711,115 @@
   Act<T> x1;
 };
 
+template <typename T> struct SEHoist {
+  int Ma;
+  const float* o_hi;
+  const float* x_hi;
+  const T* mod;
+  const int* mod_row;
+};
+
 template <typename T>
 static int se_layer(const Model& m, int wfmt, const SEW& w, const Act<T>& x, const T* c, int Mc, int mod_div, int M,
                     const std::vector<Segment>& segs, const SEBufs<T>& b, const Act<T>& out, cudaStream_t s,
-                    const std::vector<AttnPack>* packs = nullptr, const int* row_graph = nullptr) {
+                    const std::vector<AttnPack>* packs = nullptr, const int* row_graph = nullptr, const SEHoist<T>* hz = nullptr) {
   const int H = m.cfg.hidden_size, P = m.cfg.max_position_embeddings, heads = m.cfg.num_attention_heads;
-  SD_TRY(gemm_T(wfmt, Mc, H, H, c, w.ada0, w.ada0_b, 2, b.u, s));
-  SD_TRY(gemm_T(wfmt, Mc, 6 * H, H, b.u, w.ada2, w.ada2_b, 0, b.mod, s));
-  SD_TRY(gemm_T(wfmt, M, 3 * H, H, x.t, w.attn.qkv, w.attn.qkv_b, 0, b.qkv, s));
+  const int Ma = hz && hz->o_hi ? hz->Ma : M;
+  const T* mod = hz && hz->mod ? hz->mod : b.mod;
+  const int* mod_row = hz ? hz->mod_row : nullptr;
+  if (mod == b.mod) {
+    SD_TRY(gemm_T(wfmt, Mc, H, H, c, w.ada0, w.ada0_b, 2, b.u, s));
+    SD_TRY(gemm_T(wfmt, Mc, 6 * H, H, b.u, w.ada2, w.ada2_b, 0, b.mod, s));
+  }
+  SD_TRY(gemm_T(wfmt, Ma, 3 * H, H, x.t, w.attn.qkv, w.attn.qkv_b, 0, b.qkv, s));
   for (size_t gi = 0; gi < segs.size(); ++gi) {
     const Segment& g = segs[gi];
     const T* base = b.qkv + static_cast<size_t>(g.row0) * 3 * H;
     SD_TRY(attention<T>(g.B, heads, g.L, g.L, base, 3 * H, base + H, 3 * H, base + 2 * H, 3 * H, pick<T>(w.attn.E), P, g.mask,
                         b.ctx + static_cast<size_t>(g.row0) * H, s, packs ? &(*packs)[gi] : nullptr));
   }
-  SD_TRY(gemm_S(wfmt, M, H, H, b.ctx, w.attn.out, w.attn.out_b, x.s, b.o, s));
-  SD_TRY(ln_modulate<T>(b.o, M, H, true, w.attn.ln_w, w.attn.ln_b, m.cfg.layer_norm_eps, x.s, b.mod, mod_div, 0, b.x1.s, b.x1.t_out(), s, row_graph));
+  SD_TRY(gemm_S(wfmt, Ma, H, H, b.ctx, w.attn.out, w.attn.out_b, x.s, b.o, s));
+  SD_TRY(ln_modulate<T>(b.o, M, H, true, w.attn.ln_w, w.attn.ln_b, m.cfg.layer_norm_eps, x.s, mod, mod_div, 0, b.x1.s, b.x1.t_out(), s, row_graph,
+                        mod_row, Ma, hz ? hz->o_hi : nullptr, hz ? hz->x_hi : nullptr));
   SD_TRY(gemm_T(wfmt, M, 4 * H, H, b.x1.t, w.m0, w.m0_b, 1, b.m1, s));
   SD_TRY(gemm_S(wfmt, M, H, 4 * H, b.m1, w.m3, w.m3_b, nullptr, b.m2, s));
-  SD_TRY(ln_modulate<T>(b.m2, M, H, false, nullptr, nullptr, 0.f, b.x1.s, b.mod, mod_div, 3, out.s, out.t_out(), s, row_graph));
-  return SEQDIFF_OK;
+  SD_TRY(ln_modulate<T>(b.m2, M, H, false, nullptr, nullptr, 0.f, b.x1.s, mod, mod_div, 3, out.s, out.t_out(), s, row_graph, mod_row));
+  return SEQDIFF_OK;
+}
+
+template <typename T> struct FwdBufs {
+  float* te;
+  T* teT;
+  float* maskcat;
+  Act<T> x;
+  Act<T> x2;
+  SEBufs<T> sb;
+  T *ccat, *kv_all;
+  Act<T> hbuf[2];
+  float* obuf3;
+  float2* lnstats;
+  T *cq, *y, *ffn;
+};
+template <typename T>
+static FwdBufs<T> carve_forward(uint8_t* ws, cudaStream_t s, int B, int H, int I, int NL, int Mlp, int Mrp, int Ml, int Mr) {
+  constexpr bool k16 = !std::is_same<T, float>::value;
+  const size_t MtH = static_cast<size_t>(Ml + Mr) * H, MlH = static_cast<size_t>(Ml) * H;
+  Bump bp(ws, s);
+  FwdBufs<T> f;
+  f.te = bp.take<float>(static_cast<size_t>(B) * H);
+  f.teT = k16 ? bp.take<T>(static_cast<size_t>(B) * H) : reinterpret_cast<T*>(f.te);
+  f.maskcat = bp.take<float>(static_cast<size_t>(Mlp) + Mrp);
+  f.x = take_act<T>(bp, MtH);
+  f.x2 = take_act<T>(bp, MtH);
+  f.sb.x1 = take_act<T>(bp, MtH);
+  f.sb.o = bp.take<float>(MtH);
+  f.sb.m2 = bp.take<float>(MtH);
+  f.ccat = bp.take<T>(MtH);
+  f.sb.u = bp.take<T>(MtH);
+  f.sb.ctx = bp.take<T>(MtH);
+  f.sb.mod = bp.take<T>(MtH * 6);
+  f.sb.qkv = bp.take<T>(MtH * 3);
+  f.sb.m1 = bp.take<T>(MtH * 4);
+  f.kv_all = bp.take<T>(static_cast<size_t>(Mr) * NL * 2 * H);
+  f.hbuf[0] = take_act<T>(bp, MlH);
+  f.hbuf[1] = take_act<T>(bp, MlH);
+  f.obuf3 = bp.take<float>(MlH);
+  f.lnstats = bp.take<float2>(3 * static_cast<size_t>(Ml));
+  f.cq = bp.take<T>(MlH);
+  f.y = bp.take<T>(MlH);
+  f.ffn = bp.take<T>(static_cast<size_t>(Ml) * I);
+  return f;
 }
 
 
 template <typename T>
 int Model::forward_t(int wfmt, int B, int Ll, int Lr, const float* timestep, const int* step_ptr, const float* x_t,
                      const float* lig_angle, const float* lig_mask, const float* rec_seq_in, const float* rec_angle,
-                     const float* rec_mask, float* logits, cudaStream_t s, const PackInfo* pk) {
+                     const float* rec_mask, float* logits, cudaStream_t s, const PackInfo* pk, const LoopInv* inv) {
   constexpr bool k16 = !std::is_same<T, float>::value;
   const int H = cfg.hidden_size, I = cfg.intermediate_size, NL = cfg.num_hidden_layers, heads = cfg.num_attention_heads;
   const int P = cfg.max_position_embeddings;
   const float eps = cfg.layer_norm_eps;
   const int Ml = pk ? pk->Ml : B * Ll, Mr = pk ? pk->Mr : B * Lr, Mt = Ml + Mr;
   const int Mlp = B * Ll, Mrp = B * Lr;
-  const size_t MtH = static_cast<size_t>(Mt) * H, MlH = static_cast<size_t>(Ml) * H;
-  Bump bp(ws, s);
-  float* te = bp.take<float>(static_cast<size_t>(B) * H);
-  T* teT = k16 ? bp.take<T>(static_cast<size_t>(B) * H) : reinterpret_cast<T*>(te);
-  float* maskcat = bp.take<float>(static_cast<size_t>(Mlp) + Mrp);
-  Act<T> x = take_act<T>(bp, MtH);
-  Act<T> x2 = take_act<T>(bp, MtH);
-  SEBufs<T> sb;
-  sb.x1 = take_act<T>(bp, MtH);
-  sb.o = bp.take<float>(MtH);
-  sb.m2 = bp.take<float>(MtH);
-  T* ccat = bp.take<T>(MtH);
-  sb.u = bp.take<T>(MtH);
-  sb.ctx = bp.take<T>(MtH);
-  sb.mod = bp.take<T>(MtH * 6);
-  sb.qkv = bp.take<T>(MtH * 3);
-  sb.m1 = bp.take<T>(MtH * 4);
-  T* kv_all = bp.take<T>(static_cast<size_t>(Mr) * NL * 2 * H);
-  Act<T> hbuf[2] = {take_act<T>(bp, MlH), take_act<T>(bp, MlH)};
-  float* obuf3 = bp.take<float>(MlH);
-  float2* lnstats = bp.take<float2>(3 * static_cast<size_t>(Ml));
-  T* cq = bp.take<T>(MlH);
-  T* y = bp.take<T>(MlH);
-  T* ffn = bp.take<T>(static_cast<size_t>(Ml) * I);
-
-  SD_TRY(timestep_embed(timestep, step_ptr, ts_W, B, H, te, k16 ? static_cast<void*>(teT) : nullptr, Fmt<T>::v, s));
+  const size_t MlH = static_cast<size_t>(Ml) * H;
+  const FwdBufs<T> f = carve_forward<T>(ws, s, B, H, I, NL, Mlp, Mrp, Ml, Mr);
+  float* te = f.te;
+  T* teT = f.teT;
+  const Act<T> x = f.x, x2 = f.x2;
+  SEBufs<T> sb = f.sb;
+  T *ccat = f.ccat, *kv_all = f.kv_all, *cq = f.cq, *y = f.y, *ffn = f.ffn;
+  const Act<T>* hbuf = f.hbuf;
+  float2* lnstats = f.lnstats;
+
+  if (!inv) SD_TRY(timestep_embed(timestep, step_ptr, ts_W, B, H, te, k16 ? static_cast<void*>(teT) : nullptr, Fmt<T>::v, s));
   const Act<T> xr = offset(x, MlH);
   {
-    auto job = [&](const float* in, int M, const EmbW& e, const float* te_, int L, float* o32, T* oT, bool lig) {
+    const float* te_ = inv ? inv->te : te;
+    auto job = [&](const float* in, int M, const EmbW& e, bool cond, int L, float* o32, T* oT, bool lig) {
       EmbedJob jb{};
-      jb.x = in; jb.Wt = e.Wt_; jb.b = e.b; jb.lnw = e.ln_w; jb.lnb = e.ln_b; jb.te = te_;
+      jb.x = in; jb.Wt = e.Wt_; jb.b = e.b; jb.lnw = e.ln_w; jb.lnb = e.ln_b; jb.te = cond ? te_ : nullptr;
+      jb.te_row = cond && inv ? step_ptr : nullptr;
       jb.out32 = o32; jb.outT = oT; jb.M = M; jb.fin = e.fin; jb.L = L;
       if (pk) {
         jb.src_rows = lig ? pk->src_l : pk->src_r;
@@ -782,13 +828,12 @@
       return jb;
     };
     EmbedJobs jobs{};
-    jobs.n = 4;
-    jobs.j[0] = job(x_t, Ml, lig_seq, nullptr, Ll, x.s, x.t_out(), true);
-    jobs.j[1] = job(rec_seq_in, Mr, rec_seq, nullptr, Lr, xr.s, xr.t_out(), false);
-    jobs.j[2] = job(lig_angle, Ml, lig_ang, te, Ll, k16 ? nullptr : reinterpret_cast<float*>(ccat), k16 ? ccat : nullptr, true);
-    jobs.j[3] = job(rec_angle, Mr, rec_ang, te, Lr, k16 ? nullptr : reinterpret_cast<float*>(ccat + MlH), k16 ? ccat + MlH : nullptr, false);
-    if (Ll == Lr) {
-      jobs.cat_dst = maskcat; jobs.cat_a = lig_mask; jobs.cat_b = rec_mask; jobs.cat_na = Mlp; jobs.cat_nb = Mrp;
+    jobs.j[jobs.n++] = job(x_t, Ml, lig_seq, false, Ll, x.s, x.t_out(), true);
+    if (!inv) jobs.j[jobs.n++] = job(rec_seq_in, Mr, rec_seq, false, Lr, xr.s, xr.t_out(), false);
+    jobs.j[jobs.n++] = job(lig_angle, Ml, lig_ang, true, Ll, k16 ? nullptr : reinterpret_cast<float*>(ccat), k16 ? ccat : nullptr, true);
+    jobs.j[jobs.n++] = job(rec_angle, Mr, rec_ang, true, Lr, k16 ? nullptr : reinterpret_cast<float*>(ccat + MlH), k16 ? ccat + MlH : nullptr, false);
+    if (Ll == Lr && !inv) {
+      jobs.cat_dst = f.maskcat; jobs.cat_a = lig_mask; jobs.cat_b = rec_mask; jobs.cat_na = Mlp; jobs.cat_nb = Mrp;
     }
     SD_TRY(embed_ln_multi<T>(jobs, eps, H, s));
   }
@@ -797,8 +842,15 @@
   std::vector<AttnPack> packs;
   AttnPack pk_self{}, pk_cross{};
   if (pk) {
+    pk_self = AttnPack{pk->off_l, pk->off_l, pk->len_l, Ml, Ml, Ll};
+    pk_cross = AttnPack{pk->off_l, pk->off_r, pk->len_l, Ml, Mr, Lr};
+  }
+  if (inv) {
+    segs.push_back({0, B, pk ? pk->max_l : Ll, lig_mask});
+    if (pk) packs.push_back(pk_self);
+  } else if (pk) {
     if (Ll == Lr) {
-      segs.push_back({0, 2 * B, pk->max_l > pk->max_r ? pk->max_l : pk->max_r, maskcat});
+      segs.push_back({0, 2 * B, pk->max_l > pk->max_r ? pk->max_l : pk->max_r, f.maskcat});
       packs.push_back(AttnPack{pk->off_cat, pk->off_cat, pk->len_cat, Mt, Mt, Ll});
     } else {
       segs.push_back({0, B, pk->max_l, lig_mask});
@@ -806,10 +858,8 @@
       segs.push_back({0, B, pk->max_r, rec_mask});
       packs.push_back(AttnPack{pk->off_cat + B, pk->off_cat + B, pk->len_cat + B, Mt, Mt, Lr});
     }
-    pk_self = AttnPack{pk->off_l, pk->off_l, pk->len_l, Ml, Ml, Ll};
-    pk_cross = AttnPack{pk->off_l, pk->off_r, pk->len_l, Ml, Mr, Lr};
   } else if (Ll == Lr) {
-    segs.push_back({0, 2 * B, Ll, maskcat});
+    segs.push_back({0, 2 * B, Ll, f.maskcat});
   } else {
     segs.push_back({0, B, Ll, lig_mask});
     segs.push_back({Ml, B, Lr, rec_mask});
@@ -817,13 +867,14 @@
   const int Lq_self = pk ? pk->max_l : Ll, Lk_cross = pk ? pk->max_r : Lr;
   const AttnPack* aps = pk ? &pk_self : nullptr;
   const AttnPack* apc = pk ? &pk_cross : nullptr;
-  SD_TRY(se_layer<T>(*this, wfmt, se_lig, x, ccat, Mt, 1, Mt, segs, sb, x2, s, pk ? &packs : nullptr, nullptr));
+  const SEHoist<T> hz_lig{Ml, inv ? inv->o : nullptr, inv ? inv->xr : nullptr, nullptr, nullptr};
+  SD_TRY(se_layer<T>(*this, wfmt, se_lig, x, ccat, Mt, 1, Mt, segs, sb, x2, s, pk ? &packs : nullptr, nullptr, inv ? &hz_lig : nullptr));
   const T* rec = x2.t + MlH;
 
   SD_TRY(gemm_T(wfmt, Mr, NL * 2 * H, H, rec, ckv_all, ckv_all_b, 0, kv_all, s));
   Act<T> h = x2;
   if constexpr (k16) {
-    float* obuf[3] = {sb.o, sb.m2, obuf3};
+    float* obuf[3] = {sb.o, sb.m2, f.obuf3};
     LnResid prev{};
     const float* o_prev = nullptr;
     for (int i = 0; i < NL; ++i) {
@@ -877,7 +928,8 @@
   std::vector<Segment> lseg{{0, B, Lq_self, lig_mask}};
   std::vector<AttnPack> lpack;
   if (pk) lpack.push_back(pk_self);
-  SD_TRY(se_layer<T>(*this, wfmt, se_dec, h, teT, B, Ll, Ml, lseg, sb, x, s, pk ? &lpack : nullptr, pk ? pk->graph : nullptr));
+  const SEHoist<T> hz_dec{Ml, nullptr, nullptr, inv ? static_cast<const T*>(inv->mod) : nullptr, step_ptr};
+  SD_TRY(se_layer<T>(*this, wfmt, se_dec, h, teT, B, Ll, Ml, lseg, sb, x, s, pk ? &lpack : nullptr, pk ? pk->graph : nullptr, inv ? &hz_dec : nullptr));
 
   if constexpr (std::is_same<T, bf16>::value) {
     f16* xh = reinterpret_cast<f16*>(sb.ctx);
@@ -894,12 +946,13 @@
 
 int Model::forward(int precision, int B, int Ll, int Lr, const float* timestep, const int* step_ptr, const float* x_t,
                    const float* lig_angle, const float* lig_mask, const float* rec_seq_in, const float* rec_angle,
-                   const float* rec_mask, float* logits, cudaStream_t s, const PackInfo* pk) {
+                   const float* rec_mask, float* logits, cudaStream_t s, const PackInfo* pk, const LoopInv* inv) {
   SD_CHECK(finalized, "model not finalised (seqdiff_model_finalize)");
   SD_CHECK(arch == kArchSequence, "handle holds a structure model: use seqdiff_struct_forward");
   SD_CHECK(!pk || precision != SEQDIFF_FP32, "ragged packing runs in the 16-bit modes");
   SD_CHECK(precision >= SEQDIFF_FP32 && precision <= SEQDIFF_FP16, "unknown precision mode");
   SD_CHECK(B > 0 && Ll > 0 && Lr > 0, "empty batch");
+  SD_CHECK(!inv || step_ptr, "the sampling-loop invariants are indexed by the device step counter");
   if (cfg.relative_key) SD_CHECK(Ll <= cfg.max_position_embeddings && Lr <= cfg.max_position_embeddings, "Length exceed");
   SD_CUDA(cudaSetDevice(device));
   SD_TRY(ensure_workspace(workspace_need(precision, B, Ll, Lr)));
@@ -907,12 +960,39 @@
   const PdlScope pdl_scope(pdl_auto_mode(pk ? static_cast<long long>(pk->Ml) + pk->Mr : static_cast<long long>(B) * (Ll + Lr)));
   switch (precision) {
     case SEQDIFF_FP32:
-      return forward_t<float>(1, B, Ll, Lr, timestep, step_ptr, x_t, lig_angle, lig_mask, rec_seq_in, rec_angle, rec_mask, logits, s, nullptr);
+      return forward_t<float>(1, B, Ll, Lr, timestep, step_ptr, x_t, lig_angle, lig_mask, rec_seq_in, rec_angle, rec_mask, logits, s, nullptr, inv);
     case SEQDIFF_BF16:
-      return forward_t<bf16>(1, B, Ll, Lr, timestep, step_ptr, x_t, lig_angle, lig_mask, rec_seq_in, rec_angle, rec_mask, logits, s, pk);
+      return forward_t<bf16>(1, B, Ll, Lr, timestep, step_ptr, x_t, lig_angle, lig_mask, rec_seq_in, rec_angle, rec_mask, logits, s, pk, inv);
     default:
-      return forward_t<f16>(0, B, Ll, Lr, timestep, step_ptr, x_t, lig_angle, lig_mask, rec_seq_in, rec_angle, rec_mask, logits, s, pk);
-  }
+      return forward_t<f16>(0, B, Ll, Lr, timestep, step_ptr, x_t, lig_angle, lig_mask, rec_seq_in, rec_angle, rec_mask, logits, s, pk, inv);
+  }
+}
+
+template <typename T>
+int Model::loop_invariants_t(int wfmt, int B, int Ll, int Lr, int T_, const float* rec_seq_in, const float* rec_mask, const LoopInv& iv,
+                             cudaStream_t s, const PackInfo* pk) {
+  constexpr bool k16 = !std::is_same<T, float>::value;
+  const int H = cfg.hidden_size, heads = cfg.num_attention_heads, P = cfg.max_position_embeddings;
+  const int Ml = pk ? pk->Ml : B * Ll, Mr = pk ? pk->Mr : B * Lr;
+  const FwdBufs<T> f = carve_forward<T>(ws, s, B, H, cfg.intermediate_size, cfg.num_hidden_layers, B * Ll, B * Lr, Ml, Mr);
+  SD_TRY(timestep_embed(nullptr, nullptr, ts_W, T_, H, iv.te, k16 ? iv.teT : nullptr, Fmt<T>::v, s));
+  SD_TRY(gemm_T(wfmt, T_, H, H, static_cast<const T*>(iv.teT), se_dec.ada0, se_dec.ada0_b, 2, static_cast<T*>(iv.u), s));
+  SD_TRY(gemm_T(wfmt, T_, 6 * H, H, static_cast<const T*>(iv.u), se_dec.ada2, se_dec.ada2_b, 0, static_cast<T*>(iv.mod), s));
+  EmbedJobs jobs{};
+  jobs.n = 1;
+  EmbedJob& jb = jobs.j[0];
+  jb.x = rec_seq_in; jb.Wt = rec_seq.Wt_; jb.b = rec_seq.b; jb.lnw = rec_seq.ln_w; jb.lnb = rec_seq.ln_b;
+  jb.out32 = iv.xr; jb.outT = k16 ? iv.xrT : nullptr; jb.M = Mr; jb.fin = rec_seq.fin; jb.L = Lr;
+  if (pk) jb.src_rows = pk->src_r;
+  SD_TRY(embed_ln_multi<T>(jobs, cfg.layer_norm_eps, H, s));
+  const AttnW& a = se_lig.attn;
+  T* qkv = f.sb.qkv;
+  SD_TRY(gemm_T(wfmt, Mr, 3 * H, H, static_cast<const T*>(iv.xrT), a.qkv, a.qkv_b, 0, qkv, s));
+  const AttnPack ap = pk ? AttnPack{pk->off_r, pk->off_r, pk->len_r, Mr, Mr, Lr} : AttnPack{};
+  const int Lk = pk ? pk->max_r : Lr;
+  SD_TRY(attention<T>(B, heads, Lk, Lk, qkv, 3 * H, qkv + H, 3 * H, qkv + 2 * H, 3 * H, pick<T>(a.E), P, rec_mask, f.sb.ctx, s, pk ? &ap : nullptr));
+  SD_TRY(gemm_S(wfmt, Mr, H, H, f.sb.ctx, a.out, a.out_b, iv.xr, iv.o, s));
+  return SEQDIFF_OK;
 }
 
 int Model::build_pack(int B, int Ll, int Lr, const float* lig_mask, const float* rec_mask, cudaStream_t s, bool* usable) {
@@ -1041,14 +1121,41 @@
     }
   }
 
+  {
+    inv.rows = T > inv.rows ? T : inv.rows;
+    const size_t es = precision == SEQDIFF_FP32 ? 4 : 2, NrH = Nr * cfg.hidden_size, tH = static_cast<size_t>(inv.rows) * cfg.hidden_size;
+    const size_t need_inv = 2 * align256(NrH * 4) + align256(NrH * 2) + align256(tH * 4) + align256(tH * 2) + align256(tH * es) +
+                            align256(tH * 6 * es) + 8 * kGuardBytes;
+    if (need_inv > samp_inv_bytes) {
+      if (samp_inv) { SD_CUDA(cudaDeviceSynchronize()); debug_guard_begin(samp_inv); SD_CUDA(cudaFree(samp_inv)); samp_inv = nullptr; samp_inv_bytes = 0; }
+      SD_CUDA(cudaMalloc(reinterpret_cast<void**>(&samp_inv), need_inv));
+      samp_inv_bytes = need_inv;
+    }
+    Bump bi(samp_inv, s);
+    inv.xr = bi.take<float>(NrH);
+    inv.xrT = es == 2 ? static_cast<void*>(bi.take<uint16_t>(NrH)) : inv.xr;
+    inv.o = bi.take<float>(NrH);
+    inv.te = bi.take<float>(tH);
+    inv.teT = es == 2 ? static_cast<void*>(bi.take<uint16_t>(tH)) : inv.te;
+    inv.u = bi.take<uint8_t>(tH * es);
+    inv.mod = bi.take<uint8_t>(tH * 6 * es);
+    const PdlScope pdl_scope(pdl_auto_mode(pk ? static_cast<long long>(pk->Ml) + pk->Mr : static_cast<long long>(B) * (Ll + Lr)));
+    switch (precision) {
+      case SEQDIFF_FP32: SD_TRY(loop_invariants_t<float>(1, B, Ll, Lr, T, c_rseq, c_rmask, inv, s, nullptr)); break;
+      case SEQDIFF_BF16: SD_TRY(loop_invariants_t<bf16>(1, B, Ll, Lr, T, c_rseq, c_rmask, inv, s, pk)); break;
+      default: SD_TRY(loop_invariants_t<f16>(0, B, Ll, Lr, T, c_rseq, c_rmask, inv, s, pk)); break;
+    }
+  }
+
   GraphKey key;
   key.pack_hash = pk ? pk->hash : 0;
   key.precision = precision; key.B = B; key.Ll = Ll; key.Lr = Lr; key.diverse = diverse; key.noise = noise_E;
   key.ws_ptr = ws; key.in_ptr = samp_in; key.tab_ptr = d_tables;
+  key.inv_ptr = samp_inv; key.inv_rows = inv.rows;
   uint64_t* d_rng = reinterpret_cast<uint64_t*>(d_step + 16);
   auto one_step = [&](cudaStream_t st) -> int {
     const PdlScope pdl_scope(pdl_auto_mode(pk ? static_cast<long long>(pk->Ml) + pk->Mr : static_cast<long long>(B) * (Ll + Lr)));
-    SD_TRY(forward(precision, B, Ll, Lr, nullptr, d_step, x_cur, c_lang, c_lmask, c_rseq, c_rang, c_rmask, logits, st, pk));
+    SD_TRY(forward(precision, B, Ll, Lr, nullptr, d_step, x_cur, c_lang, c_lmask, c_rseq, c_rang, c_rmask, logits, st, pk, &inv));
     SD_TRY(reverse_step(d_tables, 1, B, Ll, x_cur, logits, diverse, noise_E, 0, 0, 0, d_step, x_cur, nullptr, st, d_step + 1, d_rng));
     return SEQDIFF_OK;
   };
@@ -1056,7 +1163,7 @@
     if (graph_exec) { cudaGraphExecDestroy(graph_exec); graph_exec = nullptr; }
     SD_CUDA(launch_k(set_int_kernel, dim3(1), dim3(1), 0, s, d_step, T - 1));
     SD_LAUNCHED("set_int", s);
-    SD_TRY(forward(precision, B, Ll, Lr, nullptr, d_step, x_cur, c_lang, c_lmask, c_rseq, c_rang, c_rmask, logits, s, pk));
+    SD_TRY(forward(precision, B, Ll, Lr, nullptr, d_step, x_cur, c_lang, c_lmask, c_rseq, c_rang, c_rmask, logits, s, pk, &inv));
     SD_CUDA(cudaStreamSynchronize(s));
     cudaGraph_t graph = nullptr;
     const uint64_t l0 = g_launches.load();
diff --git a/e3-invaraint-diffusion-model_b200/csrc/model.cuh b/e3-invaraint-diffusion-model_b200/csrc/model.cuh
--- a/e3-invaraint-diffusion-model_b200/csrc/model.cuh
+++ b/e3-invaraint-diffusion-model_b200/csrc/model.cuh
@@ -84,6 +84,17 @@
   uint64_t hash = 0;
 };
 
+struct LoopInv {
+  int rows = 0;
+  float* xr = nullptr;
+  void* xrT = nullptr;
+  float* o = nullptr;
+  float* te = nullptr;
+  void* teT = nullptr;
+  void* u = nullptr;
+  void* mod = nullptr;
+};
+
 enum Arch { kArchSequence = 0, kArchStructure = 1 };
 
 struct Model {
@@ -113,6 +124,9 @@
   size_t tables_cap = 0;
   uint8_t* samp_in = nullptr;
   size_t samp_in_bytes = 0;
+  uint8_t* samp_inv = nullptr;
+  size_t samp_inv_bytes = 0;
+  LoopInv inv;
   cudaGraphExec_t graph_exec = nullptr;
   int graph_kernels = 0;
   cudaStream_t loop_stream = nullptr;
@@ -124,11 +138,13 @@
     const void* in_ptr = nullptr;
     const void* tab_ptr = nullptr;
     const void* aux_ptr = nullptr;
+    const void* inv_ptr = nullptr;
+    int inv_rows = 0;
     int T = 0;
     uint64_t pack_hash = 0;
     bool operator==(const GraphKey& o) const {
       return pack_hash == o.pack_hash && aux_ptr == o.aux_ptr && T == o.T && precision == o.precision && B == o.B && Ll == o.Ll && Lr == o.Lr && diverse == o.diverse && noise == o.noise &&
-             ws_ptr == o.ws_ptr && in_ptr == o.in_ptr && tab_ptr == o.tab_ptr;
+             ws_ptr == o.ws_ptr && in_ptr == o.in_ptr && tab_ptr == o.tab_ptr && inv_ptr == o.inv_ptr && inv_rows == o.inv_rows;
     }
   } graph_key;
 
@@ -138,7 +154,7 @@
   int finalize(cudaStream_t s);
   int forward(int precision, int B, int Ll, int Lr, const float* timestep, const int* step_ptr, const float* x_t,
               const float* lig_angle, const float* lig_mask, const float* rec_seq, const float* rec_angle, const float* rec_mask,
-              float* logits, cudaStream_t s, const PackInfo* pk = nullptr);
+              float* logits, cudaStream_t s, const PackInfo* pk = nullptr, const LoopInv* inv = nullptr);
   int sample(int precision, int B, int Ll, int Lr, int T, const float* q_tables, const float* x_T, const float* lig_angle,
              const float* lig_mask, const float* rec_seq, const float* rec_angle, const float* rec_mask, int diverse,
              const float* noise_E, uint64_t seed, uint64_t gid0, float* final_out, cudaStream_t s, int flags = 0);
@@ -197,7 +213,10 @@
   template <typename T>
   int forward_t(int wfmt, int B, int Ll, int Lr, const float* timestep, const int* step_ptr, const float* x_t, const float* lig_angle,
                 const float* lig_mask, const float* rec_seq, const float* rec_angle, const float* rec_mask, float* logits,
-                cudaStream_t s, const PackInfo* pk);
+                cudaStream_t s, const PackInfo* pk, const LoopInv* inv);
+  template <typename T>
+  int loop_invariants_t(int wfmt, int B, int Ll, int Lr, int T_, const float* rec_seq, const float* rec_mask, const LoopInv& inv, cudaStream_t s,
+                        const PackInfo* pk);
 };
 
 }
diff --git a/e3-invaraint-diffusion-model_b200/csrc/rowwise.cu b/e3-invaraint-diffusion-model_b200/csrc/rowwise.cu
--- a/e3-invaraint-diffusion-model_b200/csrc/rowwise.cu
+++ b/e3-invaraint-diffusion-model_b200/csrc/rowwise.cu
@@ -46,7 +46,7 @@
   const int i = blockIdx.x * blockDim.x + threadIdx.x;
   if (i >= B * half) return;
   const int b = i / half, j = i % half;
-  const float t = step_ptr ? static_cast<float>(*step_ptr) : timestep[b];
+  const float t = step_ptr ? static_cast<float>(*step_ptr) : (timestep ? timestep[b] : static_cast<float>(b));
   const float x = __fmul_rn(__fmul_rn(__fmul_rn(t, W[j]), 2.0f), 3.14159274101257324f);
   const float sv = sinf(x), cv = cosf(x);
   out[static_cast<size_t>(b) * H + j] = sv;
@@ -157,7 +157,8 @@
       }
       float mean, rstd;
       row_stats<VPL>(v, H, eps, mean, rstd);
-      const float* terow = job.te ? job.te + static_cast<size_t>(job.row_graph ? __ldg(job.row_graph + tok0 + t) : (tok0 + t) / job.L) * H : nullptr;
+      const int te_r = job.te_row ? *job.te_row : (job.row_graph ? __ldg(job.row_graph + tok0 + t) : (tok0 + t) / job.L);
+      const float* terow = job.te ? job.te + static_cast<size_t>(te_r) * H : nullptr;
 #pragma unroll
       for (int i = 0; i < VPL; ++i) {
         float g8[8], b8[8];
@@ -293,14 +294,17 @@
 __global__ void __launch_bounds__(kRowThreads) ln_modulate_kernel(const float* __restrict__ in, int M, int H, const float* __restrict__ lnw,
                                                                   const float* __restrict__ lnb, float eps1, const float* __restrict__ x,
                                                                   const T* __restrict__ mod, int mod_div, int chunk0,
-                                                                  float* __restrict__ out32, T* __restrict__ outT, const int* __restrict__ row_graph) {
+                                                                  float* __restrict__ out32, T* __restrict__ outT, const int* __restrict__ row_graph,
+                                                                  const int* __restrict__ mod_row, int split, const float* __restrict__ in_hi,
+                                                                  const float* __restrict__ x_hi) {
   pdl_trigger();
   pdl_wait();
   const int lane = threadIdx.x & 31;
   const int row = (blockIdx.x * kRowThreads + threadIdx.x) >> 5;
   if (row >= M) return;
+  const bool hi = in_hi && row >= split;
   float v[VPL][8];
-  load_row<float, VPL>(in + static_cast<size_t>(row) * H, lane, v);
+  load_row<float, VPL>(hi ? in_hi + static_cast<size_t>(row - split) * H : in + static_cast<size_t>(row) * H, lane, v);
   float mean, rstd;
   if (AFFINE_FIRST) {
     row_stats<VPL>(v, H, eps1, mean, rstd);
@@ -315,8 +319,10 @@
   }
   row_stats<VPL>(v, H, 1e-5f, mean, rstd);
   SD_DEV_ASSERT(!row_graph || __ldg(row_graph + row) >= 0);
-  const T* mrow = mod + static_cast<size_t>(row_graph ? __ldg(row_graph + row) : row / mod_div) * (6 * H);
-  const float* xrow = x + static_cast<size_t>(row) * H;
+  SD_DEV_ASSERT(!mod_row || *mod_row >= 0);
+  const int mr = mod_row ? *mod_row : (row_graph ? __ldg(row_graph + row) : row / mod_div);
+  const T* mrow = mod + static_cast<size_t>(mr) * (6 * H);
+  const float* xrow = hi ? x_hi + static_cast<size_t>(row - split) * H : x + static_cast<size_t>(row) * H;
 #pragma unroll
   for (int i = 0; i < VPL; ++i) {
     const int e = (i * 32 + lane) * 8;
@@ -337,18 +343,23 @@
 
 template <typename T>
 int ln_modulate(const float* in, int M, int H, bool affine_first, const float* lnw, const float* lnb, float eps1, const float* x,
-                const T* mod, int mod_div, int chunk0, float* out32, T* outT, cudaStream_t s, const int* row_graph) {
+                const T* mod, int mod_div, int chunk0, float* out32, T* outT, cudaStream_t s, const int* row_graph, const int* mod_row, int split,
+                const float* in_hi, const float* x_hi) {
+  SD_CHECK(!in_hi == !x_hi && (!in_hi || (split >= 0 && split <= M)), "ln_modulate: split sources need both in_hi and x_hi and 0 <= split <= M");
   const int grid = ceil_div(M * 32, kRowThreads);
   if (affine_first) {
-    SD_VPL_DISPATCH(H, SD_CUDA(launch_k(ln_modulate_kernel<T, VPL, true>, dim3(grid), dim3(kRowThreads), 0, s, in, M, H, lnw, lnb, eps1, x, mod, mod_div, chunk0, out32, outT, row_graph)));
+    SD_VPL_DISPATCH(H, SD_CUDA(launch_k(ln_modulate_kernel<T, VPL, true>, dim3(grid), dim3(kRowThreads), 0, s, in, M, H, lnw, lnb, eps1, x, mod, mod_div, chunk0, out32, outT, row_graph,
+                                        mod_row, split, in_hi, x_hi)));
   } else {
-    SD_VPL_DISPATCH(H, SD_CUDA(launch_k(ln_modulate_kernel<T, VPL, false>, dim3(grid), dim3(kRowThreads), 0, s, in, M, H, lnw, lnb, eps1, x, mod, mod_div, chunk0, out32, outT, row_graph)));
+    SD_VPL_DISPATCH(H, SD_CUDA(launch_k(ln_modulate_kernel<T, VPL, false>, dim3(grid), dim3(kRowThreads), 0, s, in, M, H, lnw, lnb, eps1, x, mod, mod_div, chunk0, out32, outT, row_graph,
+                                        mod_row, split, in_hi, x_hi)));
   }
   SD_LAUNCHED("ln_modulate", s);
   return SEQDIFF_OK;
 }
-#define SD_INST_LNMOD(T) \
-  template int ln_modulate<T>(const float*, int, int, bool, const float*, const float*, float, const float*, const T*, int, int, float*, T*, cudaStream_t, const int*)
+#define SD_INST_LNMOD(T)                                                                                                                                  \
+  template int ln_modulate<T>(const float*, int, int, bool, const float*, const float*, float, const float*, const T*, int, int, float*, T*, cudaStream_t, \
+                              const int*, const int*, int, const float*, const float*)
 SD_INST_LNMOD(float);
 SD_INST_LNMOD(bf16);
 SD_INST_LNMOD(f16);
```

Result: faster. 35230 (median of 6 runs) (+4.7%).
